# shanjiayao/PTT

Measured on AMD Instinct MI355X. Metric: tracklet frames/sec (hot path: PointNet++ SA stack + Point-Track-Transformer blocks), higher is better.
Workload: dtype f32

## Files before the change

### include/ptt_hip.h

```cpp
#ifndef PTT_HIP_H
#define PTT_HIP_H

#include <stddef.h>
#include <stdint.h>

#ifdef __cplusplus
extern "C" {
#endif

#define PTT_ABI_VERSION 26

enum {
    PTT_OK = 0,
    PTT_EINVAL = -1,
    PTT_EUNSUPPORTED = -2,
    PTT_ELAUNCH = -3,
    PTT_EWORKSPACE = -4
};

typedef void* ptt_stream_t;

int ptt_version(void);
const char* ptt_error_name(int code);
const char* ptt_last_error_string(void);

int ptt_fps_f32(const float* xyz, int B, int N, int npoint, int32_t* idx_out,
                ptt_stream_t stream);
int ptt_fps_ws_f32(const float* xyz, int B, int N, int npoint, int32_t* idx_out, float* workspace,
                   size_t workspace_elems, ptt_stream_t stream);

int ptt_gather_f32(const float* feat, const int32_t* idx, int B, int C, int N, int M,
                   float* out, ptt_stream_t stream);
int ptt_gather_grad_f32(const float* grad_out, const int32_t* idx, int B, int C, int N,
                        int M, float* grad_feat, ptt_stream_t stream);

int ptt_select_centres_f32(const float* xyz, const int32_t* idx, int B, int N, int M, float* new_xyz,
                           int64_t* idx64_out, ptt_stream_t stream);

int ptt_ball_query_f32(const float* new_xyz, const float* xyz, int B, int M, int N,
                       float radius, int nsample, int32_t* idx_out, ptt_stream_t stream);

int ptt_centres_ball_query_f32(const float* xyz, const int32_t* sel, int B, int N, int M, float radius, int nsample,
                               float* new_xyz, int64_t* idx64_out, int32_t* idx_out, ptt_stream_t stream);

int ptt_group_f32(const float* feat, const int32_t* idx, int B, int C, int N, int M,
                  int ns, float* out, ptt_stream_t stream);
int ptt_group_grad_f32(const float* grad_out, const int32_t* idx, int B, int C, int N,
                       int M, int ns, float* grad_feat, ptt_stream_t stream);

size_t ptt_scatter_add_det_workspace(int B, int N, int E);
int ptt_scatter_add_det_f32(const float* src, const int32_t* idx, int B, int C, int N, int E, float* out,
                            void* workspace, size_t workspace_bytes, ptt_stream_t stream);

int ptt_knn_f32(const float* xyz, int B, int N, int k, int32_t* idx_out,
                ptt_stream_t stream);
int ptt_knn_rel_f32(const float* xyz, int B, int N, int k, int32_t* idx_out, float* rel_out,
                    ptt_stream_t stream);

size_t ptt_packed_weight_elems(int Cout, int K);
int ptt_pack_weight_f32(const float* W, int Cout, int K, float* packed,
                        ptt_stream_t stream);
int ptt_pack_weight_rot_f32(const float* W, int Cout, int K, int rot, float* packed,
                            ptt_stream_t stream);

int ptt_linear_f32(const float* X, int rows, int K, int ldx, const float* Wpacked, int Cout,
                   const float* scale, const float* shift, int relu, const float* residual,
                   int ldr, float* out, int ldo, ptt_stream_t stream);

#define PTT_SA_MAX_LAYERS 4

typedef struct ptt_sa_layer {
    const float* Wpacked;
    const float* scale;
    const float* shift;
    int Cin;
    int Cout;
    int relu;
} ptt_sa_layer;

int ptt_rows_mlp_f32(const float* X, int rows, int K, int ldx, const ptt_sa_layer* layers, int n_layers,
                     const float* residual, int ldr, float* out, int ldo, ptt_stream_t stream);

size_t ptt_ball_query_grid_workspace(int B, int N);
int ptt_ball_query_grid_f32(const float* new_xyz, const float* xyz, int B, int M, int N, float radius, int nsample,
                            int32_t* idx_out, void* workspace, size_t workspace_bytes, ptt_stream_t stream);
int ptt_centres_ball_query_grid_f32(const float* xyz, const int32_t* sel, int B, int N, int M, float radius, int nsample,
                                    float* new_xyz, int64_t* idx64_out, int32_t* idx_out, void* workspace, size_t workspace_bytes,
                                    ptt_stream_t stream);
int ptt_fps_ball_knn_f32(const float* xyz, int B, int N, int M, float radius, int nsample, int k, int32_t* inds,
                         int64_t* inds64, float* new_xyz, int32_t* idx, int32_t* knn, float* rel, ptt_stream_t stream);
#define PTT_POINT_JOBS_MAX 4
typedef struct ptt_point_job {
    const float* xyz; const int32_t* centre_sel; const int32_t* point_sel;
    float* new_xyz; int64_t* idx64_out; int32_t* idx_out; float* rel_out;
    int32_t kind, sel_ld, B, Nraw, Npts, M, nsample;
    float radius;
} ptt_point_job;
int ptt_point_jobs_f32(const ptt_point_job* jobs, int n_jobs, ptt_stream_t stream);

#define PTT_ROW_JOBS_MAX 4
typedef struct ptt_row_job {
    const float* X; const float* X2;
    const float* Xmax;
    const float* Wpacked; const float* scale; const float* shift;
    const float* res; const float* res2;
    float* out; float* out2; float* raw;
    const float* rel; const float* w1;
    const float* qkv; const int32_t* knn; const float* pos;
    int32_t rows, K, K1, ldx, ldx2, Cout;
    int32_t act, res_split, ldr, ldr2, out_split, out_col0, ldo, ldo2, ldraw;
    int32_t prologue, epilogue, ldq, q_off, k_off, v_off, ldp, N;
    float sm_scale;
// ... 264 lines not shown
    const float* gamma; const float* beta;
    float* act_a; float* act_b;
    float* running_mean; float* running_var;
    int64_t* num_batches_tracked;
    float momentum;
} ptt_bn_train_tail;
int ptt_bn_stats_train_f32(const float* X, int R, int C, int ldx, float eps, float* mean, float* var, float* invstd,
                           void* workspace, size_t workspace_bytes, const ptt_bn_train_tail* tail, ptt_stream_t stream);
int ptt_bn_finish_partials_train_f32(const double* partial, int chunks, int C, int R, float eps, float* mean, float* var,
                                     float* invstd, const ptt_bn_train_tail* tail, ptt_stream_t stream);
typedef struct ptt_pack_job {
    const float* W;
    int64_t out_offset, stride_out, stride_k;
    int32_t Cout, K;
} ptt_pack_job;
int ptt_pack_weights_f32(const ptt_pack_job* jobs_device, int n_jobs, float* arena, ptt_stream_t stream);
size_t ptt_linear_wgrad2_workspace(int R, int Cout, int Cin);
int ptt_linear_wgrad2_f32(const float* dZ, int ldz, const float* X, int ldx, int R, int Cout, int Cin, float* dW,
                          int accumulate, void* workspace, size_t workspace_bytes, const float* x_scale, const float* x_shift,
                          ptt_stream_t stream);

typedef struct ptt_track_loss_desc {
    const float* seed_cls;
    const float* cls_label;
    const int64_t* search_inds;
    const float* votes;
    const float* reg_label;
    const float* box_data;
    const float* centres;
    const float* pos_weight_seed;
    const float* pos_weight_box;
    int32_t B, N, Ns, M, ld_reg;
    float w_seed_cls, w_seed_reg, w_box_cls, w_box_reg;
} ptt_track_loss_desc;
int ptt_track_losses_f32(const ptt_track_loss_desc* desc, float* out8, float* total , ptt_stream_t stream);
int ptt_track_losses_bwd_f32(const ptt_track_loss_desc* desc, const float* out8, const float* upstream, float* d_seed_cls,
                             float* d_votes, float* d_box_data, ptt_stream_t stream);
typedef struct ptt_adam_tensor {
    float* param;
    float* grad;
    float* exp_avg;
    float* exp_avg_sq;
    int64_t n;
} ptt_adam_tensor;
typedef struct ptt_adam_hyper {
    float beta1, beta2, one_minus_beta1, one_minus_beta2 , eps, step_size, bias2_sqrt,
          weight_decay, max_norm;
    int32_t write_clipped;
} ptt_adam_hyper;
int ptt_adam_chunk_elems(void);
int ptt_adam_clip_step_f32(const ptt_adam_tensor* tensors_device, const int32_t* chunk_tensor_device, const int64_t* chunk_first_device,
                           int n_chunks, const ptt_adam_hyper* hyper, double* partial, size_t partial_elems, float* norm_out,
                           ptt_stream_t stream);
int ptt_adam_clip_step_dev_f32(const ptt_adam_tensor* tensors_device, const int32_t* chunk_tensor_device, const int64_t* chunk_first_device,
                               int n_chunks, const ptt_adam_hyper* hyper_device, int clip, double* partial, size_t partial_elems,
                               float* norm_out, ptt_stream_t stream);
int ptt_unit_rows_f32(const float* x, long long sb, long long sn, long long sc, int B, int n, int C, float eps, float* unit, float* nrm,
                      ptt_stream_t stream);
int ptt_cos_bwd_rows_f32(const float* A, const float* unit, const float* nrm, const float* G, const float* cosm, long long map_sb,
                         long long own, long long other, int m, int B, int n, int C, float* dx, long long sb, long long sn, long long sc,
                         ptt_stream_t stream);
size_t ptt_sa_z0_bnbwd_workspace(long long R, int C);
int ptt_sa_z0_bnbwd_f32(const double* partial, int chunks, const float* G, const float* Z0, const float* rel_rows, const float* mean,
                        const float* invstd, const float* gamma, const float* act_scale, const float* act_shift, long long R, int C,
                        float* dz_out, float* dwx, float* dgamma, float* dbeta, void* workspace, size_t workspace_bytes, ptt_stream_t stream);

typedef struct ptt_grad_job {
    const float* partial;
    int32_t nchunks, reserved;
} ptt_grad_job;
typedef struct ptt_grad_segment {
    int64_t dst;
    int32_t n, cols, ld, job0, njobs, out, vec, reserved;
} ptt_grad_segment;
int ptt_linear_wgrad_partials_f32(const float* dZ, int ldz, const float* X, int ldx, int R, int Cout, int Cin, void* workspace,
                                  size_t workspace_bytes, const float* x_scale, const float* x_shift, int* nchunks, ptt_stream_t stream);
int ptt_linear_wgrad2_partials_f32(const float* dZ, int ldz, const float* X, int ldx, int R, int Cout, int Cin, void* workspace,
                                   size_t workspace_bytes, const float* x_scale, const float* x_shift, int* nchunks, ptt_stream_t stream);
int ptt_colsum_partials_f32(const float* X, int R, int C, int ldx, void* workspace, size_t workspace_bytes, int* nchunks,
                            ptt_stream_t stream);
int ptt_grad_finish_f32(const ptt_grad_segment* segments_device, const ptt_grad_job* jobs_device, const int32_t* blocks_device,
                        int n_blocks, float* flat, ptt_stream_t stream);

int ptt_rows_gemm_rsum16_supported(int rows, int K, int N, int ldx);
int ptt_rows_gemm_rsum16_f32(const float* X, int rows, int K, int ldx, const float* Wpacked, int N, const float* residual, int ldr,
                             float* out, int ldo, float* plain, int ldp, float* gsum, int ldg, ptt_stream_t stream);
int ptt_scatter_rows_csr_sub_f32(const float* g, const int32_t* order, const int32_t* start, int B, int N, int E, int C,
                                 const float* minuend, float* out, ptt_stream_t stream);

int ptt_layernorm_train_fwd_f32(const float* x, int rows, int C, int ldx, const float* weight, const float* bias, float eps,
                                const float* residual, int ldr, float* out, int ldo, float* mean, float* rstd, ptt_stream_t stream);
size_t ptt_layernorm_bwd_workspace(int rows, int C);
int ptt_layernorm_bwd_f32(const float* dy, int ldg, const float* x, int ldx, const float* mean, const float* rstd, const float* weight,
                          int rows, int C, float* dx, int ldd, float* dweight, float* dbias, void* workspace, size_t workspace_bytes,
                          ptt_stream_t stream);
int ptt_rows_gemm_rsum16_heads_supported(int rows, int D, int hd, int ldx);
int ptt_rows_gemm_rsum16_heads_f32(const float* X, int rows, int D, int hd, int ldx, const float* Wpacked, const float* residual, int ldr,
                                   float* out, int ldo, float* plain, int ldp, float* gsum, int ldg, ptt_stream_t stream);

#ifdef __cplusplus
}
#endif
#endif
```

### ptt_amd/_lib.py

```python
import ctypes
import os
import re
from ctypes import Structure, c_char_p, c_double, c_float, c_int, c_int32, c_int64, c_longlong, c_size_t, c_uint32, c_void_p

from .build import HEADER as HEADER_PATH, LIB as LIB_PATH


def _strip_comments(text):
    return re.sub(r"/\*.*?\*/|//[^\n]*", " ", text, flags=re.S)


def parse_defines(text):
    return {n: int(v) for n, v in re.findall(r"^[ \t]*#[ \t]*define[ \t]+(PTT_\w+)[ \t]+(-?\d+)[ \t]*$", _strip_comments(text), re.M)}


CTYPES = {"int": c_int, "int32_t": c_int32, "uint32_t": c_uint32, "int64_t": c_int64, "long long": c_longlong, "size_t": c_size_t,
          "float": c_float, "double": c_double, "ptt_stream_t": c_void_p}


def _ctype(decl, name, is_return=False):
    words = decl.replace("*", " * ").split()
    if not is_return and len(words) > 1 and words[-1] != "*":
        words.pop()
    if "*" in words:
# ... 34 lines not shown

_header = _read_header()
PROTOTYPES = parse_prototypes(_header)
EXPORTS = list(PROTOTYPES)
DEFINES = parse_defines(_header)
ABI_VERSION = DEFINES["PTT_ABI_VERSION"]
PTT_SA_MAX_LAYERS = DEFINES["PTT_SA_MAX_LAYERS"]
PTT_MAX_SEGMENTS = DEFINES["PTT_MAX_SEGMENTS"]
PTT_CROP_JOBS_BY_VALUE_MAX = DEFINES["PTT_CROP_JOBS_BY_VALUE_MAX"]


class CropJob(Structure):
    _fields_ = [("points", c_void_p), ("ld", c_int64),
                ("lo1", c_double * 3), ("hi1", c_double * 3), ("trans", c_double * 3), ("rot", c_double * 9),
                ("lo2", c_double * 3), ("hi2", c_double * 3),
                ("out", c_void_p), ("count", c_void_p), ("n_points", c_int32), ("capacity", c_int32),
                ("label_out", c_void_p), ("ltrans", c_double * 3), ("lrot", c_double * 9), ("llo", c_double * 3), ("lhi", c_double * 3),
                ("append", c_int32), ("reserved", c_int32)]


class RegularizeJob(Structure):
    _fields_ = [("seg", c_void_p * PTT_MAX_SEGMENTS), ("seg_count", c_void_p * PTT_MAX_SEGMENTS),
                ("seg_capacity", c_int32 * PTT_MAX_SEGMENTS), ("out", c_void_p), ("info", c_void_p),
                ("n_seg", c_int32), ("input_size", c_int32)]


class TrackBox(Structure):
    _fields_ = [("center", c_double * 3), ("wlh", c_double * 3), ("quat", c_double * 4)]


class BnTrainTail(Structure):
    _fields_ = [("gamma", c_void_p), ("beta", c_void_p), ("act_a", c_void_p), ("act_b", c_void_p),
                ("running_mean", c_void_p), ("running_var", c_void_p), ("num_batches_tracked", c_void_p), ("momentum", c_float)]


class BnBwdInput(Structure):
    _fields_ = [("g", c_void_p), ("ldg", c_int), ("arg", c_void_p), ("ns", c_int), ("z", c_void_p), ("ldz", c_int),
                ("k1", c_void_p), ("c0", c_void_p), ("c1", c_void_p), ("mean", c_void_p), ("act_a", c_void_p), ("act_b", c_void_p),
                ("dz_out", c_void_p), ("ldd", c_int)]


class PackJob(Structure):
    _fields_ = [("W", c_void_p), ("out_offset", c_int64), ("stride_out", c_int64), ("stride_k", c_int64),
                ("Cout", c_int32), ("K", c_int32)]


class RowJob(Structure):
    _fields_ = [("X", c_void_p), ("X2", c_void_p), ("Xmax", c_void_p), ("Wpacked", c_void_p), ("scale", c_void_p), ("shift", c_void_p),
                ("res", c_void_p), ("res2", c_void_p), ("out", c_void_p), ("out2", c_void_p), ("raw", c_void_p),
                ("rel", c_void_p), ("w1", c_void_p), ("qkv", c_void_p), ("knn", c_void_p), ("pos", c_void_p),
                ("rows", c_int32), ("K", c_int32), ("K1", c_int32), ("ldx", c_int32), ("ldx2", c_int32), ("Cout", c_int32),
                ("act", c_int32), ("res_split", c_int32), ("ldr", c_int32), ("ldr2", c_int32), ("out_split", c_int32),
                ("out_col0", c_int32), ("ldo", c_int32), ("ldo2", c_int32), ("ldraw", c_int32),
                ("prologue", c_int32), ("epilogue", c_int32), ("ldq", c_int32), ("q_off", c_int32), ("k_off", c_int32),
                ("v_off", c_int32), ("ldp", c_int32), ("N", c_int32), ("sm_scale", c_float), ("col_tiles", c_int32),
                ("idx", c_void_p), ("xyz", c_void_p), ("centres", c_void_p), ("wx", c_void_p), ("radius", c_float),
                ("ns", c_int32), ("M", c_int32), ("normalize_xyz", c_int32), ("pro_relu", c_int32)]


class PointJob(Structure):
    _fields_ = [("xyz", c_void_p), ("centre_sel", c_void_p), ("point_sel", c_void_p), ("new_xyz", c_void_p), ("idx64_out", c_void_p),
                ("idx_out", c_void_p), ("rel_out", c_void_p), ("kind", c_int32), ("sel_ld", c_int32), ("B", c_int32),
                ("Nraw", c_int32), ("Npts", c_int32), ("M", c_int32), ("nsample", c_int32), ("radius", c_float)]


class TrackLossDesc(Structure):
    _fields_ = [("seed_cls", c_void_p), ("cls_label", c_void_p), ("search_inds", c_void_p), ("votes", c_void_p), ("reg_label", c_void_p),
                ("box_data", c_void_p), ("centres", c_void_p), ("pos_weight_seed", c_void_p), ("pos_weight_box", c_void_p),
                ("B", c_int32), ("N", c_int32), ("Ns", c_int32), ("M", c_int32), ("ld_reg", c_int32),
                ("w_seed_cls", c_float), ("w_seed_reg", c_float), ("w_box_cls", c_float), ("w_box_reg", c_float)]


class AdamTensor(Structure):
    _fields_ = [("param", c_void_p), ("grad", c_void_p), ("exp_avg", c_void_p), ("exp_avg_sq", c_void_p), ("n", c_int64)]


class GradJob(Structure):
    _fields_ = [("partial", c_void_p), ("nchunks", c_int32), ("reserved", c_int32)]


class GradSegment(Structure):
    _fields_ = [("dst", c_int64), ("n", c_int32), ("cols", c_int32), ("ld", c_int32), ("job0", c_int32), ("njobs", c_int32), ("out", c_int32),
                ("vec", c_int32), ("reserved", c_int32)]


class AdamHyper(Structure):
    _fields_ = [("beta1", c_float), ("beta2", c_float), ("one_minus_beta1", c_float), ("one_minus_beta2", c_float), ("eps", c_float), ("step_size", c_float), ("bias2_sqrt", c_float),
                ("weight_decay", c_float), ("max_norm", c_float), ("write_clipped", c_int32)]


class SaLayer(Structure):
    _fields_ = [("Wpacked", c_void_p), ("scale", c_void_p), ("shift", c_void_p),
                ("Cin", c_int), ("Cout", c_int), ("relu", c_int)]


class SaDesc(Structure):
    _fields_ = [("xyz", c_void_p), ("new_xyz", c_void_p), ("idx", c_void_p), ("feat", c_void_p),
                ("feat_sb", c_int64), ("feat_sc", c_int64), ("feat_sn", c_int64),
                ("out", c_void_p), ("out_sb", c_int64), ("out_sc", c_int64), ("out_sm", c_int64),
                ("B", c_int), ("N", c_int), ("M", c_int), ("nsample", c_int), ("C", c_int),
                ("radius", c_float), ("use_xyz", c_int), ("normalize_xyz", c_int), ("n_layers", c_int),
                ("layers", SaLayer * PTT_SA_MAX_LAYERS),
                ("l0_point_term", c_void_p), ("l0_xyz_weight", c_void_p), ("l0_channels", c_int), ("l0_relu", c_int),
                ("compact_ws", c_void_p), ("compact_ws_bytes", c_size_t)]


class XcorrDesc(Structure):
    _fields_ = [("cos_t", c_void_p), ("P", c_void_p), ("w_sim", c_void_p), ("scale0", c_void_p), ("shift0", c_void_p),
                ("out", c_void_p), ("out_sb", c_int64), ("out_sc", c_int64), ("out_sn", c_int64),
                ("sim_out", c_void_p),
                ("B", c_int), ("Ns", c_int), ("Nt", c_int), ("C0", c_int),
                ("n_layers", c_int), ("layers", SaLayer * PTT_SA_MAX_LAYERS),
                ("split", c_int32), ("out_sh", c_int64), ("search_feat", c_void_p), ("templ_feat", c_void_p),
                ("s_sb", c_int64), ("s_sn", c_int64), ("t_sb", c_int64), ("t_sn", c_int64), ("C", c_int), ("eps", c_float)]


class AttnDesc(Structure):
    _fields_ = [("xyz", c_void_p), ("rel", c_void_p), ("knn", c_void_p), ("qkv", c_void_p),
                ("Wd1p", c_void_p), ("Wd2p", c_void_p), ("bd2", c_void_p),
                ("Wg1p", c_void_p), ("bg1", c_void_p), ("Wg2p", c_void_p), ("bg2", c_void_p),
                ("res", c_void_p), ("attn", c_void_p),
                ("B", c_int), ("N", c_int), ("k", c_int), ("D", c_int), ("order", c_void_p), ("heads", c_int)]


_lib = None


def lib():
    global _lib
    if _lib is None:
        if not os.path.exists(LIB_PATH):
            raise RuntimeError(
                "ptt_amd: %s is missing — build it with `python -m ptt_amd.build` "
                "(hipcc --offload-arch=gfx950); there is no CPU fallback" % LIB_PATH)
        import torch
        try:
            loaded = ctypes.CDLL(LIB_PATH)
        except OSError as e:
            raise RuntimeError("ptt_amd: cannot load %s: %s" % (LIB_PATH, e))
        for name, (restype, argtypes) in PROTOTYPES.items():
            fn = getattr(loaded, name)
            fn.restype, fn.argtypes = restype, argtypes
        if loaded.ptt_version() != ABI_VERSION:
            raise RuntimeError("ptt_amd: %s has ABI version %d, this package expects %d — rebuild it with "
                               "`python -m ptt_amd.build`" % (LIB_PATH, loaded.ptt_version(), ABI_VERSION))
        _lib = loaded
    return _lib


def check(rc, what):
    if rc != 0:
        l = lib()
        raise RuntimeError("%s failed: %s (%s)" % (what, l.ptt_error_name(rc).decode(),
                                                   l.ptt_last_error_string().decode()))
```

### ptt_amd/csrc/point_ops.hip

```cpp
#pragma clang fp contract(off)

#include <limits.h>
#include <stdlib.h>
#include "common.h"

namespace ptt {

__device__ __forceinline__ float sqdist3(float ax, float ay, float az, float bx, float by, float bz) {
    const float dx = ax - bx, dy = ay - by, dz = az - bz;
    return (dx * dx + dy * dy) + dz * dz;
}

__device__ __forceinline__ float knn_dist(float ax, float ay, float az, float bx, float by, float bz) {
    const float d = sqdist3(ax, ay, az, bx, by, bz);
    return d < __builtin_inff() ? d : 3.402823466e+38f;
}

__device__ __forceinline__ float lane_bcast(float v, int src_lane) {
    return __builtin_bit_cast(float, __builtin_amdgcn_readlane(__builtin_bit_cast(int, v), src_lane));
}

typedef float fps_f2 __attribute__((ext_vector_type(2)));


template <int T, int P, bool LX, int ABL = 0>
__global__ __launch_bounds__(T) void fps_kernel(const float* __restrict__ xyz, int N, int npoint,
                                               int32_t* __restrict__ idx_out) {
    constexpr int W = T / 64;
    const int b = blockIdx.x;
    const float* __restrict__ pts = xyz + (size_t)b * N * 3;
    int32_t* __restrict__ out = idx_out + (size_t)b * npoint;
    const int t = threadIdx.x;
    const int lane = t & 63;
    const int wv = t >> 6;

    extern __shared__ int sel_lds[];
    float* xyz_lds = reinterpret_cast<float*>(sel_lds + ((npoint + 3) & ~3));

    float px[P], py[P], pz[P], md[P];
#pragma unroll
    for (int i = 0; i < P; ++i) {
        const int k = t * P + i;
        float x = 0.f, y = 0.f, z = 0.f, m = -1.0f;
        if (k < N) {
            x = pts[3 * k + 0];
            y = pts[3 * k + 1];
            z = pts[3 * k + 2];
            const float mag = (x * x + y * y) + z * z;
            m = (mag > 1e-3f) ? 1e10f : -1.0f;
            if (LX) { xyz_lds[3 * k + 0] = x; xyz_lds[3 * k + 1] = y; xyz_lds[3 * k + 2] = z; }
        }
        px[i] = x; py[i] = y; pz[i] = z; md[i] = m;
    }

    __shared__ __attribute__((aligned(16))) float slots[2][W > 1 ? W : 1][8];

    float lx = pts[0], ly = pts[1], lz = pts[2];
    if (t == 0 && npoint > 0) sel_lds[0] = 0;
    if (LX) __syncthreads();

    for (int j = 1; j < npoint; ++j) {
        float best = -1.0f, bx = 0.f, by = 0.f, bz = 0.f;
        int besti = 0;
        if constexpr ((P % 2) == 0) {
            const fps_f2 lxv = {lx, lx}, lyv = {ly, ly}, lzv = {lz, lz};
#pragma unroll
            for (int i = 0; i < ((ABL & 32) ? 2 : P); i += 2) {
                const fps_f2 dx = fps_f2{px[i], px[i + 1]} - lxv, dy = fps_f2{py[i], py[i + 1]} - lyv,
                             dz = fps_f2{pz[i], pz[i + 1]} - lzv;
                const fps_f2 d = (dx * dx + dy * dy) + dz * dz;
#pragma unroll
                for (int h = 0; h < 2; ++h) {
                    const float m = fminf(md[i + h], d[h]);
                    md[i + h] = m;
                    const bool take = m > best;
                    best = take ? m : best;
                    besti = take ? t * P + i + h : besti;
                    if (!LX) {
                        bx = take ? px[i + h] : bx;
                        by = take ? py[i + h] : by;
                        bz = take ? pz[i + h] : bz;
                    }
                }
            }
        } else {
#pragma unroll
            for (int i = 0; i < P; ++i) {
                const float d = sqdist3(px[i], py[i], pz[i], lx, ly, lz);
                const float m = fminf(md[i], d);
                md[i] = m;
                const bool take = m > best;
                best = take ? m : best;
                besti = take ? t * P + i : besti;
                if (!LX) {
                    bx = take ? px[i] : bx;
                    by = take ? py[i] : by;
                    bz = take ? pz[i] : bz;
                }
            }
        }
        float wmax;
        if constexpr (ABL & 1) wmax = __builtin_amdgcn_readfirstlane(best); else wmax = wave_max_f32_fused(best);
        int src;
        if constexpr (ABL & 2) {
            src = (int)(__builtin_bit_cast(unsigned, wmax) & 63u);
        } else {
            const unsigned long long winners = __ballot(best == wmax);
            src = __ffsll((long long)winners) - 1;
            if constexpr (ABL & 1) src &= 63;
        }
        if constexpr (W == 1) {
            int widx = __builtin_amdgcn_readlane(besti, src);
// ... 2 lines not shown
                lx = (float)widx * 1e-3f; ly = lx; lz = lx;
            } else if constexpr (LX) {
                lx = xyz_lds[3 * widx + 0]; ly = xyz_lds[3 * widx + 1]; lz = xyz_lds[3 * widx + 2];
            } else if (wmax < 0.f) {
                lx = pts[0]; ly = pts[1]; lz = pts[2];
            } else {
                lx = lane_bcast(bx, src); ly = lane_bcast(by, src); lz = lane_bcast(bz, src);
            }
            if (lane == 0) sel_lds[j] = widx;
        } else if constexpr ((ABL & 4) != 0) {
            int gi = __builtin_amdgcn_readlane(besti, src);
            if (wmax < 0.f) gi = 0;
            if constexpr ((ABL & 8) != 0) { lx = (float)gi * 1e-3f; ly = lx; lz = lx; }
            else { lx = xyz_lds[3 * gi + 0]; ly = xyz_lds[3 * gi + 1]; lz = xyz_lds[3 * gi + 2]; }
            if (lane == 0 && wv == 0) sel_lds[j] = gi;
        } else {
            const int par = j & 1;
            if (lane == src) {
                if constexpr (LX) {
                    *reinterpret_cast<float2*>(slots[par][wv]) = make_float2(best, __builtin_bit_cast(float, besti));
                } else {
                    float4* s4 = reinterpret_cast<float4*>(slots[par][wv]);
                    s4[0] = make_float4(best, __builtin_bit_cast(float, besti), bx, by);
                    slots[par][wv][4] = bz;
                }
            }
            if constexpr ((ABL & 16) == 0) __syncthreads();
            float gd, gx = 0.f, gy = 0.f, gz = 0.f;
            int gi;
            if constexpr (W <= 4) {
                gd = -1.0f; gi = 0;
#pragma unroll
                for (int w = 0; w < W; ++w) {
                    if constexpr (LX) {
                        const float2 s2 = *reinterpret_cast<const float2*>(slots[par][w]);
                        const bool take = s2.x > gd;
                        gd = take ? s2.x : gd;
                        gi = take ? __builtin_bit_cast(int, s2.y) : gi;
                    } else {
                        const float4 s4 = *reinterpret_cast<const float4*>(slots[par][w]);
                        const float sz = slots[par][w][4];
                        const bool take = s4.x > gd;
                        gd = take ? s4.x : gd;
                        gi = take ? __builtin_bit_cast(int, s4.y) : gi;
                        gx = take ? s4.z : gx;
                        gy = take ? s4.w : gy;
                        gz = take ? sz : gz;
                    }
                }
            } else {
                if constexpr (LX) {
                    float2 s2 = make_float2(-1.0f, 0.f);
                    if (lane < W) s2 = *reinterpret_cast<const float2*>(slots[par][lane]);
                    gd = wave_max_f32_fused(s2.x);
                    const int sl = __ffsll((long long)__ballot(s2.x == gd)) - 1;
                    gi = __builtin_amdgcn_readlane(__builtin_bit_cast(int, s2.y), sl);
                } else {
                    float4 s4 = make_float4(-1.0f, 0.f, 0.f, 0.f);
                    float sz = 0.f;
                    if (lane < W) { s4 = *reinterpret_cast<const float4*>(slots[par][lane]); sz = slots[par][lane][4]; }
                    gd = wave_max_f32_fused(s4.x);
                    const int sl = __ffsll((long long)__ballot(s4.x == gd)) - 1;
                    gi = __builtin_amdgcn_readlane(__builtin_bit_cast(int, s4.y), sl);
                    gx = lane_bcast(s4.z, sl); gy = lane_bcast(s4.w, sl); gz = lane_bcast(sz, sl);
                }
            }
            if (gd < 0.f) gi = 0;
            if constexpr ((ABL & 16) != 0) gi &= 1023;
            if constexpr ((ABL & 8) != 0) {
                lx = (float)gi * 1e-3f; ly = lx; lz = lx;
            } else if constexpr (LX) {
                lx = xyz_lds[3 * gi + 0]; ly = xyz_lds[3 * gi + 1]; lz = xyz_lds[3 * gi + 2];
            } else {
                if (gd < 0.f) { gx = pts[0]; gy = pts[1]; gz = pts[2]; }
                lx = gx; ly = gy; lz = gz;
            }
            if (t == 0) sel_lds[j] = gi;
        }
    }
    __syncthreads();
    for (int j = t; j < npoint; j += T) out[j] = sel_lds[j];
}

template <int T, int P>
static int launch_fps(const float* xyz, int B, int N, int npoint, int32_t* idx, hipStream_t s) {
    const size_t sel_bytes = (size_t)((npoint + 3) & ~3) * sizeof(int);
    if (sel_bytes + (size_t)N * 12 + 1024 <= 65536 && !dev_switches().fps_plain) {
#ifdef PTT_DEV
        if (const char* e = getenv("PTT_FPS_ABL")) {
            const int abl = atoi(e);
#define PTT_FPS_ABL_CASE(A) if (abl == A) { hipLaunchKernelGGL((fps_kernel<T, P, true, A>), dim3(B), dim3(T), sel_bytes + (size_t)N * 12, s, xyz, N, npoint, idx); return check_launch("fps_kernel(abl)"); }
            PTT_FPS_ABL_CASE(1) PTT_FPS_ABL_CASE(2) PTT_FPS_ABL_CASE(3) PTT_FPS_ABL_CASE(4) PTT_FPS_ABL_CASE(8) PTT_FPS_ABL_CASE(12) PTT_FPS_ABL_CASE(15)
            PTT_FPS_ABL_CASE(16) PTT_FPS_ABL_CASE(32) PTT_FPS_ABL_CASE(47) PTT_FPS_ABL_CASE(7) PTT_FPS_ABL_CASE(24) PTT_FPS_ABL_CASE(40)
#undef PTT_FPS_ABL_CASE
        }
#endif
        hipLaunchKernelGGL((fps_kernel<T, P, true>), dim3(B), dim3(T), sel_bytes + (size_t)N * 12, s, xyz, N, npoint, idx);
        return check_launch("fps_kernel");
    }
    hipLaunchKernelGGL((fps_kernel<T, P, false>), dim3(B), dim3(T), sel_bytes, s, xyz, N, npoint, idx);
    return check_launch("fps_kernel");
}

template <int CPW>
__device__ __forceinline__ void ball_sweep(const float* __restrict__ pts, int N, float r2, int ns, const float (&cx)[CPW],
                                           const float (&cy)[CPW], const float (&cz)[CPW], int ncentres,
                                           int32_t* __restrict__ out0, int lane) {
    int cnt[CPW], first[CPW];
#pragma unroll
    for (int c = 0; c < CPW; ++c) { cnt[c] = (c < ncentres) ? 0 : ns; first[c] = 0; }
    for (int base = 0; base < N; base += 64) {
        const int k = base + lane;
        const bool in = k < N;
        float px = 0.f, py = 0.f, pz = 0.f;
        if (in) { px = pts[3 * k + 0]; py = pts[3 * k + 1]; pz = pts[3 * k + 2]; }
        bool active = false;
#pragma unroll
        for (int c = 0; c < CPW; ++c) {
            if (cnt[c] >= ns) continue;
            const float d = sqdist3(cx[c], cy[c], cz[c], px, py, pz);
            const bool hit = in && d < r2;
            const unsigned long long mask = __ballot(hit);
            if (mask != 0ull) {
                if (cnt[c] == 0) first[c] = base + (__ffsll((long long)mask) - 1);
                const int pos = cnt[c] + __popcll(mask & ((1ull << lane) - 1ull));
                if (hit && pos < ns) out0[(size_t)c * ns + pos] = k;
                cnt[c] += __popcll(mask);
            }
            active = active || cnt[c] < ns;
        }
        if (!active) break;
    }
#pragma unroll
    for (int c = 0; c < CPW; ++c) {
        if (c >= ncentres) break;
        const int fill = (cnt[c] > 0) ? first[c] : 0;
        for (int s = cnt[c] + lane; s < ns; s += 64) out0[(size_t)c * ns + s] = fill;
    }
}

template <int CPW>
__global__ __launch_bounds__(256) void ball_query_kernel(const float* __restrict__ new_xyz,
                                                         const float* __restrict__ xyz, int BM, int M, int N,
                                                         float r2, int ns, int32_t* __restrict__ idx_out) {
    const int centre = (blockIdx.x * 4 + (threadIdx.x >> 6)) * CPW;
    if (centre >= BM) return;
    const int lane = threadIdx.x & 63;
    const int b = centre / M;
    float cx[CPW], cy[CPW], cz[CPW];
    const int nc = min(CPW, BM - centre);
#pragma unroll
    for (int c = 0; c < CPW; ++c) {
        const int cc = centre + (c < nc ? c : 0);
        cx[c] = new_xyz[(size_t)cc * 3 + 0]; cy[c] = new_xyz[(size_t)cc * 3 + 1]; cz[c] = new_xyz[(size_t)cc * 3 + 2];
    }
    ball_sweep<CPW>(xyz + (size_t)b * N * 3, N, r2, ns, cx, cy, cz, nc, idx_out + (size_t)centre * ns, lane);
}

template <int CPW>
__global__ __launch_bounds__(256) void centres_ball_query_kernel(const float* __restrict__ xyz, const int32_t* __restrict__ sel,
                                                                 int BM, int M, int N, float r2, int ns,
                                                                 float* __restrict__ new_xyz, long long* __restrict__ idx64,
                                                                 int32_t* __restrict__ idx_out) {
    const int centre = (blockIdx.x * 4 + (threadIdx.x >> 6)) * CPW;
    if (centre >= BM) return;
    const int lane = threadIdx.x & 63;
// ... 691 lines not shown
            const int s0 = cstart[c0], s1 = cstart[c0 + (x1 - x0) + 1];
            for (int e = s0 + lane; e < s1; e += 64) {
                const int k = cpts[e];
                const float d = sqdist3(cx, cy, cz, pts[3 * k], pts[3 * k + 1], pts[3 * k + 2]);
                if (d < r2) atomicOr(&bits[k >> 5], 1u << (k & 31));
            }
        }
    }
    __builtin_amdgcn_wave_barrier();
    asm volatile("s_waitcnt lgkmcnt(0)" ::: "memory");
    int32_t* __restrict__ out = idx_out + (size_t)centre * ns;
    int cnt = 0, first = 0;
    for (int w0 = 0; w0 < words && cnt < ns; w0 += 64) {
        const int w = w0 + lane;
        unsigned v = w < words ? bits[w] : 0u;
        const int mine = __popc(v);
        int incl = mine;
#pragma unroll
        for (int off = 1; off < 64; off <<= 1) { const int u = __shfl_up(incl, off, 64); if (lane >= off) incl += u; }
        const int total = __shfl(incl, 63, 64);
        if (total == 0) continue;
        if (cnt == 0) {
            const unsigned long long any = __ballot(mine > 0);
            const int fl = __ffsll((long long)any) - 1;
            const unsigned fv = __shfl(v, fl, 64);
            first = ((w0 + fl) << 5) + (__ffs(fv) - 1);
        }
        int pos = cnt + incl - mine;
        while (v != 0u && pos < ns) {
            const int bit = __ffs(v) - 1;
            out[pos++] = (w << 5) + bit;
            v &= v - 1u;
        }
        cnt += total;
    }
    const int have = cnt < ns ? cnt : ns;
    const int fill = cnt > 0 ? first : 0;
    for (int s2 = have + lane; s2 < ns; s2 += 64) out[s2] = fill;
}

}

using namespace ptt;

extern "C" int ptt_fps_f32(const float* xyz, int B, int N, int npoint, int32_t* idx_out, ptt_stream_t stream) {
    if (B < 0 || N <= 0 || npoint < 0) return fail(PTT_EINVAL, "ptt_fps_f32: B=%d N=%d npoint=%d", B, N, npoint);
    if (B == 0 || npoint == 0) return PTT_OK;
    if (!xyz || !idx_out) return fail(PTT_EINVAL, "ptt_fps_f32: null pointer");
    if (npoint > 15360) return fail(PTT_EUNSUPPORTED, "ptt_fps_f32: npoint=%d exceeds the LDS index buffer (15360)", npoint);
    hipStream_t s = as_stream(stream);
    if (N <= 64) return launch_fps<64, 1>(xyz, B, N, npoint, idx_out, s);
    if (N <= 128) return launch_fps<64, 2>(xyz, B, N, npoint, idx_out, s);
    if (N <= 256) return launch_fps<64, 4>(xyz, B, N, npoint, idx_out, s);
    if (N <= 512) {
        if (const int T = dev_switches().fps_t) {
            if (T == 256) return launch_fps<256, 2>(xyz, B, N, npoint, idx_out, s);
            if (T == 128) return launch_fps<128, 4>(xyz, B, N, npoint, idx_out, s);
            if (T == 512) return launch_fps<512, 1>(xyz, B, N, npoint, idx_out, s);
        }
        return launch_fps<64, 8>(xyz, B, N, npoint, idx_out, s);
    }
    if (N <= 1024) {
        if (const int T = dev_switches().fps_t) {
            if (T == 64) return launch_fps<64, 16>(xyz, B, N, npoint, idx_out, s);
            if (T == 128) return launch_fps<128, 8>(xyz, B, N, npoint, idx_out, s);
            if (T == 512) return launch_fps<512, 2>(xyz, B, N, npoint, idx_out, s);
        }
        return launch_fps<256, 4>(xyz, B, N, npoint, idx_out, s);
    }
    if (N <= 2048) {
        if (const int T = dev_switches().fps_t) {
            if (T == 512) return launch_fps<512, 4>(xyz, B, N, npoint, idx_out, s);
            if (T == 1024) return launch_fps<1024, 2>(xyz, B, N, npoint, idx_out, s);
            if (T == 128) return launch_fps<128, 16>(xyz, B, N, npoint, idx_out, s);
        }
        return launch_fps<256, 8>(xyz, B, N, npoint, idx_out, s);
    }
    if (N <= 4096) return launch_fps<512, 8>(xyz, B, N, npoint, idx_out, s);
    if (N <= 8192) return launch_fps<1024, 8>(xyz, B, N, npoint, idx_out, s);
    if (N <= 16384) return launch_fps<1024, 16>(xyz, B, N, npoint, idx_out, s);
    return fail(PTT_EUNSUPPORTED, "ptt_fps_f32: N=%d exceeds the register-resident limit 16384 (use ptt_fps_ws_f32)", N);
}

extern "C" int ptt_spatial_order_f32(const float* xyz, int B, int N, int32_t* order, ptt_stream_t stream) {
    if (B < 0 || N <= 0) return fail(PTT_EINVAL, "ptt_spatial_order_f32: B=%d N=%d", B, N);
    if (B == 0) return PTT_OK;
    if (!xyz || !order) return fail(PTT_EINVAL, "ptt_spatial_order_f32: null pointer");
    if (N > 8192 || (long long)B * N > INT_MAX) return fail(PTT_EUNSUPPORTED, "ptt_spatial_order_f32: N=%d (at most 8192 points per cloud are sorted in LDS)", N);
    int P = 2;
    while (P < N) P <<= 1;
    const int lds = P * (int)sizeof(unsigned long long);
    if (int rc = set_lds_limit(reinterpret_cast<const void*>(spatial_order_kernel), lds)) return rc;
    hipLaunchKernelGGL(spatial_order_kernel, dim3(B), dim3(1024), lds, as_stream(stream), xyz, N, P, order);
    return check_launch("spatial_order_kernel");
}

extern "C" int ptt_fps_ws_f32(const float* xyz, int B, int N, int npoint, int32_t* idx_out, float* workspace, size_t workspace_elems,
                              ptt_stream_t stream) {
    if (B < 0 || N <= 0 || npoint < 0) return fail(PTT_EINVAL, "ptt_fps_ws_f32: B=%d N=%d npoint=%d", B, N, npoint);
    if (B == 0 || npoint == 0) return PTT_OK;
    if (!xyz || !idx_out) return fail(PTT_EINVAL, "ptt_fps_ws_f32: null pointer");
    if ((long long)N * 3 > INT_MAX) return fail(PTT_EUNSUPPORTED, "ptt_fps_ws_f32: N=%d", N);
    if (!workspace || workspace_elems < (size_t)B * N)
        return fail(PTT_EWORKSPACE, "ptt_fps_ws_f32: %zu floats of workspace needed", (size_t)B * N);
    hipLaunchKernelGGL(fps_ws_kernel, dim3(B), dim3(1024), 0, as_stream(stream), xyz, N, npoint, workspace, idx_out);
    return check_launch("fps_ws_kernel");
}

static int ball_cpw(int BM, int M) {
    const int force = dev_switches().ball_cpw;
    if (force == 1 || (M & 3) != 0) return 1;
    if (force == 8 && (M & 7) == 0) return 8;
    if (force == 4) return 4;
    return BM >= 4 * 256 * 8 ? 4 : 1;
}

extern "C" int ptt_ball_query_f32(const float* new_xyz, const float* xyz, int B, int M, int N, float radius,
                                  int nsample, int32_t* idx_out, ptt_stream_t stream) {
    if (B < 0 || M < 0 || N <= 0 || nsample <= 0)
        return fail(PTT_EINVAL, "ptt_ball_query_f32: B=%d M=%d N=%d nsample=%d", B, M, N, nsample);
    if (B == 0 || M == 0) return PTT_OK;
    if (!new_xyz || !xyz || !idx_out) return fail(PTT_EINVAL, "ptt_ball_query_f32: null pointer");
    const float r2 = radius * radius;
    const int BM = B * M;
    const int cpw = ball_cpw(BM, M);
    if (cpw == 8)
        hipLaunchKernelGGL((ball_query_kernel<8>), dim3((BM / 8 + 3) / 4), dim3(256), 0, as_stream(stream), new_xyz, xyz, BM, M,
                           N, r2, nsample, idx_out);
    else if (cpw == 4)
        hipLaunchKernelGGL((ball_query_kernel<4>), dim3((BM / 4 + 3) / 4), dim3(256), 0, as_stream(stream), new_xyz, xyz, BM, M,
                           N, r2, nsample, idx_out);
    else
        hipLaunchKernelGGL((ball_query_kernel<1>), dim3((BM + 3) / 4), dim3(256), 0, as_stream(stream), new_xyz, xyz, BM, M,
                           N, r2, nsample, idx_out);
    return check_launch("ball_query_kernel");
}

extern "C" int ptt_gather_f32(const float* feat, const int32_t* idx, int B, int C, int N, int M, float* out,
                              ptt_stream_t stream) {
    if (B < 0 || C < 0 || N <= 0 || M < 0) return fail(PTT_EINVAL, "ptt_gather_f32: bad sizes");
    const size_t total = (size_t)B * C * M;
    if (total == 0) return PTT_OK;
    if (!feat || !idx || !out) return fail(PTT_EINVAL, "ptt_gather_f32: null pointer");
    hipLaunchKernelGGL(gather_kernel, dim3(grid_for(total, 256)), dim3(256), 0, as_stream(stream), feat, idx, C, N, M,
                       out, total);
    return check_launch("gather_kernel");
}

extern "C" int ptt_select_centres_f32(const float* xyz, const int32_t* idx, int B, int N, int M, float* new_xyz,
                                      int64_t* idx64_out, ptt_stream_t stream) {
    if (B < 0 || N <= 0 || M < 0 || (!idx && M > N)) return fail(PTT_EINVAL, "ptt_select_centres_f32: B=%d N=%d M=%d", B, N, M);
    const size_t total = (size_t)B * M;
    if (total == 0) return PTT_OK;
    if (!xyz || !new_xyz) return fail(PTT_EINVAL, "ptt_select_centres_f32: null pointer");
    hipLaunchKernelGGL(select_centres_kernel, dim3(grid_for(total, 256)), dim3(256), 0, as_stream(stream), xyz, idx, N, M,
                       new_xyz, reinterpret_cast<long long*>(idx64_out), total);
    return check_launch("select_centres_kernel");
}

extern "C" int ptt_gather_grad_f32(const float* grad_out, const int32_t* idx, int B, int C, int N, int M,
                                   float* grad_feat, ptt_stream_t stream) {
    if (B < 0 || C < 0 || N <= 0 || M < 0) return fail(PTT_EINVAL, "ptt_gather_grad_f32: bad sizes");
    const size_t nout = (size_t)B * C * N;
    if (nout == 0) return PTT_OK;
    if (!grad_feat) return fail(PTT_EINVAL, "ptt_gather_grad_f32: null pointer");
    if (hipMemsetAsync(grad_feat, 0, nout * sizeof(float), as_stream(stream)) != hipSuccess)
// ... 216 lines not shown
```

### ptt_amd/csrc/train_ops.hip

```cpp
#include <math.h>
#include "common.h"

namespace ptt {

typedef float f32x4t __attribute__((ext_vector_type(4)));
typedef float f32x16t __attribute__((ext_vector_type(16)));

constexpr int ST_ROWS = 2048;

template <int MODE>
__global__ __launch_bounds__(256) void col_stats_kernel(const float* __restrict__ X, const float* __restrict__ Act,
                                                        const float* __restrict__ Z, const float* __restrict__ mean,
                                                        const float* __restrict__ invstd, int R, int C, int ldx, int lda,
                                                        int ldz, double* __restrict__ partial) {
    __shared__ double red[2][4][64];
    const int lane = threadIdx.x & 63, rg = threadIdx.x >> 6;
    const int r0 = blockIdx.x * ST_ROWS, r1 = min(R, r0 + ST_ROWS);
    for (int cg = 0; cg * 64 < C; ++cg) {
        const int c = cg * 64 + lane;
        double s0 = 0.0, s1 = 0.0;
        if (c < C) {
            float mu = 0.f, is = 0.f;
            if (MODE == 1) { mu = mean[c]; is = invstd[c]; }
            for (int r = r0 + rg; r < r1; r += 4) {
// ... 575 lines not shown
        const float sa = act_a ? act_a[c] : 1.f, sb = act_a ? act_b[c] : 0.f;
        float m = act_a ? fmaxf(__builtin_fmaf(p[0], sa, sb), 0.f) : p[0];
        int a = 0;
        for (int k = 1; k < ns; ++k) {
            float v = p[(size_t)k * ldx];
            if (act_a) v = fmaxf(__builtin_fmaf(v, sa, sb), 0.f);
            if (v > m) { m = v; a = k; }
        }
        out[(size_t)g * ldo + c] = m;
        arg[(size_t)g * C + c] = a;
    }
}

__global__ __launch_bounds__(256) void pool_select_kernel(const float* __restrict__ pmax, const float* __restrict__ pmin,
                                                          const int32_t* __restrict__ amax, const int32_t* __restrict__ amin,
                                                          const float* __restrict__ act_a, const float* __restrict__ act_b, size_t total,
                                                          int C, float* __restrict__ out, int32_t* __restrict__ arg) {
    for (size_t e = (size_t)blockIdx.x * 256 + threadIdx.x; e < total; e += (size_t)gridDim.x * 256) {
        const int c = (int)(e % C);
        const float a = act_a[c], b = act_b[c];
        const float y = a > 0.f ? pmax[e] : pmin[e];
        out[e] = fmaxf(__builtin_fmaf(y, a, b), 0.f);
        arg[e] = a > 0.f ? amax[e] : (a < 0.f ? amin[e] : 0);
    }
}

__global__ __launch_bounds__(256) void pool_rows_bwd_kernel(const float* __restrict__ dOut, int ldo, const int32_t* __restrict__ arg,
                                                            int G, int ns, int C, float* __restrict__ dX, int ldx) {
    const size_t total = (size_t)G * ns * C;
    for (size_t e = (size_t)blockIdx.x * 256 + threadIdx.x; e < total; e += (size_t)gridDim.x * 256) {
        const size_t row = e / C;
        const int c = (int)(e - row * C);
        const int g = (int)(row / ns), k = (int)(row - (size_t)g * ns);
        dX[row * ldx + c] = (arg[(size_t)g * C + c] == k) ? dOut[(size_t)g * ldo + c] : 0.f;
    }
}

constexpr int WG_KC = 32;
constexpr int WG_LD = 132;
constexpr int WG_ROWS = 4096;
constexpr int WG_MIN_ROWS = 64;

template <bool VEC>
__device__ __forceinline__ void wg_fetch(const float* __restrict__ P, int ld, int r0, int rmax, int c0, int cmax, int t,
                                         f32x4t (&st)[4]) {
#pragma unroll
    for (int i = 0; i < 4; ++i) {
        const int e = t + i * 256;
        const int r = r0 + (e >> 5), c = c0 + ((e & 31) << 2);
        f32x4t v = {0.f, 0.f, 0.f, 0.f};
        if (r < rmax) {
            const float* src = P + (size_t)r * ld + c;
            if (VEC && c + 3 < cmax) {
                v = *reinterpret_cast<const f32x4t*>(src);
            } else {
#pragma unroll
                for (int q = 0; q < 4; ++q)
                    if (c + q < cmax) v[q] = src[q];
            }
        }
        st[i] = v;
    }
}
__device__ __forceinline__ void wg_stage(float* S, int t, const f32x4t (&st)[4]) {
#pragma unroll
    for (int i = 0; i < 4; ++i) {
        const int e = t + i * 256;
        *reinterpret_cast<f32x4t*>(S + (e >> 5) * WG_LD + ((e & 31) << 2)) = st[i];
    }
}

__device__ __forceinline__ void wg_act(f32x4t (&st)[4], const float* __restrict__ xa, const float* __restrict__ xb, int c0, int cmax,
                                       int t) {
    const int c = c0 + ((t & 31) << 2);
    if (c + 3 < cmax) {
        const f32x4t a4 = *reinterpret_cast<const f32x4t*>(xa + c), b4 = *reinterpret_cast<const f32x4t*>(xb + c);
#pragma unroll
        for (int i = 0; i < 4; ++i)
#pragma unroll
            for (int q = 0; q < 4; ++q) st[i][q] = fmaxf(__builtin_fmaf(st[i][q], a4[q], b4[q]), 0.f);
    }
}

template <bool VZ, bool VX, int NS = 1>
__global__ __launch_bounds__(256, 2) void linear_wgrad_kernel(const float* __restrict__ dZ, int ldz, const float* __restrict__ X,
                                                              int ldx, int R, int Cout, int Cin, int nbi, int chunk_rows,
                                                              float* __restrict__ partial, const float* __restrict__ xa,
                                                              const float* __restrict__ xb, int narrow_o = 0, int narrow_i = 0) {
    extern __shared__ __attribute__((aligned(16))) float wg_smem[];
    constexpr int WG_BUF = WG_KC * WG_LD;
#define As(b) (wg_smem + (b) * WG_BUF)
#define Bs(b) (wg_smem + (2 + (b)) * WG_BUF)
    const int t = threadIdx.x, lane = t & 63, w = t >> 6, half = lane >> 5, col = lane & 31;
    const int bo = blockIdx.x / nbi, bi = blockIdx.x - bo * nbi;
    const int o0 = bo * 128, i0 = bi * 128;
    const int r_begin = blockIdx.y * chunk_rows, r_end = min(R, r_begin + chunk_rows);
    int wo = (w >> 1) * 64, wi = (w & 1) * 64;
    int sidx = 0;
    if constexpr (NS > 1) {
        if (narrow_o) { sidx = w >> 1; wo = 0; }
        if (narrow_i) { sidx = sidx * 2 + (w & 1); wi = 0; }
        sidx = __builtin_amdgcn_readfirstlane(sidx);
    }
    f32x16t acc[2][2];
#pragma unroll
    for (int a = 0; a < 2; ++a)
#pragma unroll
        for (int b = 0; b < 2; ++b)
#pragma unroll
            for (int r = 0; r < 16; ++r) acc[a][b][r] = 0.f;
    f32x4t sa[4], sb[4];
    wg_fetch<VZ>(dZ, ldz, r_begin, r_end, o0, Cout, t, sa);
    wg_fetch<VX>(X, ldx, r_begin, r_end, i0, Cin, t, sb);
    if (xa) wg_act(sb, xa, xb, i0, Cin, t);
    wg_stage(As(0), t, sa);
    wg_stage(Bs(0), t, sb);
    __syncthreads();
    int buf = 0;
    for (int r0 = r_begin; r0 < r_end; r0 += WG_KC) {
        const bool more = r0 + WG_KC < r_end;
        if (more) {
            wg_fetch<VZ>(dZ, ldz, r0 + WG_KC, r_end, o0, Cout, t, sa);
            wg_fetch<VX>(X, ldx, r0 + WG_KC, r_end, i0, Cin, t, sb);
            if (xa) wg_act(sb, xa, xb, i0, Cin, t);
        }
        const float* A = As(buf) + (half + sidx * (WG_KC / NS)) * WG_LD + wo + col;
        const float* B = Bs(buf) + (half + sidx * (WG_KC / NS)) * WG_LD + wi + col;
        float fa[2][2], fb[2][2];
        fa[0][0] = A[0]; fa[0][1] = A[32]; fb[0][0] = B[0]; fb[0][1] = B[32];
#pragma unroll
        for (int j = 0; j < WG_KC / 2 / NS; ++j) {
            const int s = j & 1;
            if (j + 1 < WG_KC / 2 / NS) {
                fa[s ^ 1][0] = A[2 * (j + 1) * WG_LD]; fa[s ^ 1][1] = A[2 * (j + 1) * WG_LD + 32];
                fb[s ^ 1][0] = B[2 * (j + 1) * WG_LD]; fb[s ^ 1][1] = B[2 * (j + 1) * WG_LD + 32];
            }
            __builtin_amdgcn_sched_barrier(0);
            acc[0][0] = __builtin_amdgcn_mfma_f32_32x32x2f32(fa[s][0], fb[s][0], acc[0][0], 0, 0, 0);
            acc[0][1] = __builtin_amdgcn_mfma_f32_32x32x2f32(fa[s][0], fb[s][1], acc[0][1], 0, 0, 0);
            acc[1][0] = __builtin_amdgcn_mfma_f32_32x32x2f32(fa[s][1], fb[s][0], acc[1][0], 0, 0, 0);
            acc[1][1] = __builtin_amdgcn_mfma_f32_32x32x2f32(fa[s][1], fb[s][1], acc[1][1], 0, 0, 0);
            __builtin_amdgcn_sched_barrier(0);
        }
        if (more) {
            wg_stage(As(buf ^ 1), t, sa);
            wg_stage(Bs(buf ^ 1), t, sb);
        }
        __syncthreads();
        buf ^= 1;
    }
#undef As
#undef Bs
    if constexpr (NS > 1) {
        float* slot = wg_smem + w * 4096;
#pragma unroll
        for (int a = 0; a < 2; ++a)
#pragma unroll
            for (int b = 0; b < 2; ++b)
#pragma unroll
                for (int r = 0; r < 16; ++r) slot[((a * 2 + b) * 16 + r) * 64 + lane] = acc[a][b][r];
        __syncthreads();
        if (sidx != 0) return;
        const int step = (NS == 4) ? 1 : (narrow_i ? 1 : 2);
        float* P = partial + (size_t)blockIdx.y * Cout * Cin;
        for (int a = 0; a < 2; ++a)
            for (int b = 0; b < 2; ++b) {
                const int ci = i0 + wi + b * 32 + col;
#pragma unroll
                for (int r = 0; r < 16; ++r) {
                    const int e = ((a * 2 + b) * 16 + r) * 64 + lane;
                    float v = slot[e];
                    for (int k = 1; k < NS; ++k) v += wg_smem[(w + k * step) * 4096 + e];
                    const int co = o0 + wo + a * 32 + (r & 3) + 8 * (r >> 2) + 4 * half;
                    if (co < Cout && ci < Cin) P[(size_t)co * Cin + ci] = v;
                }
            }
        return;
    }
    float* P = partial + (size_t)blockIdx.y * Cout * Cin;
#pragma unroll
    for (int a = 0; a < 2; ++a)
#pragma unroll
        for (int b = 0; b < 2; ++b) {
            const int ci = i0 + wi + b * 32 + col;
#pragma unroll
            for (int r = 0; r < 16; ++r) {
                const int co = o0 + wo + a * 32 + (r & 3) + 8 * (r >> 2) + 4 * half;
                if (co < Cout && ci < Cin) P[(size_t)co * Cin + ci] = acc[a][b][r];
            }
        }
}

__global__ __launch_bounds__(256) void colsum_partial_scalar_kernel(const float* __restrict__ X, int ldx, int R, int C, int rows_per_chunk,
                                                                    float* __restrict__ partial) {
    __shared__ float red[4][64];
    const int c = blockIdx.y * 64 + (threadIdx.x & 63), rg = threadIdx.x >> 6;
    const int r0 = blockIdx.x * rows_per_chunk, r1 = min(R, r0 + rows_per_chunk);
    float acc = 0.f;
    if (c < C)
        for (int r = r0 + rg; r < r1; r += 4) acc += X[(size_t)r * ldx + c];
    red[rg][threadIdx.x & 63] = acc;
    __syncthreads();
    if (rg == 0 && c < C) partial[(size_t)blockIdx.x * C + c] = ((red[0][threadIdx.x] + red[1][threadIdx.x]) + red[2][threadIdx.x]) + red[3][threadIdx.x];
}

constexpr int WK_ROWS = 256;
template <int K>
__global__ __launch_bounds__(256) void wgrad_smallk_kernel(const float* __restrict__ dZ, int ldz, const float* __restrict__ X, int ldx,
                                                           int R, int C, float* __restrict__ partial) {
    __shared__ float red[256][4 * K];
    const int Cq = C >> 2, span = Cq < 256 ? Cq : 256, RG = 256 / span;
    const int q0 = threadIdx.x % span, rg = threadIdx.x / span;
    const int r0 = blockIdx.x * WK_ROWS, r1 = min(R, r0 + WK_ROWS);
    for (int qb = 0; qb < Cq; qb += span) {
        const int q = qb + q0;
        float acc[4][K];
#pragma unroll
        for (int j = 0; j < 4; ++j)
#pragma unroll
            for (int k = 0; k < K; ++k) acc[j][k] = 0.f;
        if (q < Cq && rg < RG) {
            for (int r = r0 + rg; r < r1; r += RG) {
                const f32x4t g = *reinterpret_cast<const f32x4t*>(dZ + (size_t)r * ldz + 4 * q);
                float xv[K];
#pragma unroll
                for (int k = 0; k < K; ++k) xv[k] = X[(size_t)r * ldx + k];
#pragma unroll
                for (int j = 0; j < 4; ++j)
#pragma unroll
                    for (int k = 0; k < K; ++k) acc[j][k] = __builtin_fmaf(g[j], xv[k], acc[j][k]);
            }
        }
#pragma unroll
        for (int j = 0; j < 4; ++j)
#pragma unroll
            for (int k = 0; k < K; ++k) red[threadIdx.x][j * K + k] = acc[j][k];
        __syncthreads();
        if (rg == 0 && q < Cq) {
#pragma unroll
            for (int j = 0; j < 4; ++j)
#pragma unroll
                for (int k = 0; k < K; ++k) {
                    float t = 0.f;
                    for (int g2 = 0; g2 < RG; ++g2) t += red[g2 * span + q0][j * K + k];
                    partial[((size_t)blockIdx.x * C + 4 * q + j) * K + k] = t;
                }
        }
        __syncthreads();
    }
}

constexpr int CS_ROWS = 128;
__global__ __launch_bounds__(256) void colsum_partial_kernel(const float* __restrict__ X, int ldx, int R, int C, int rows_per_chunk,
                                                             float* __restrict__ partial) {
    __shared__ f32x4t red[4][64];
    const int q = blockIdx.y * 64 + (threadIdx.x & 63), rg = threadIdx.x >> 6;
    const int r0 = blockIdx.x * rows_per_chunk, r1 = min(R, r0 + rows_per_chunk);
    f32x4t acc = {0.f, 0.f, 0.f, 0.f};
    if (4 * q < C) {
        int r = r0 + rg;
        for (; r + 12 < r1; r += 16) {
            const f32x4t a = *reinterpret_cast<const f32x4t*>(X + (size_t)r * ldx + 4 * q);
            const f32x4t b = *reinterpret_cast<const f32x4t*>(X + (size_t)(r + 4) * ldx + 4 * q);
            const f32x4t c = *reinterpret_cast<const f32x4t*>(X + (size_t)(r + 8) * ldx + 4 * q);
            const f32x4t d = *reinterpret_cast<const f32x4t*>(X + (size_t)(r + 12) * ldx + 4 * q);
#pragma unroll
            for (int k = 0; k < 4; ++k) acc[k] = (((acc[k] + a[k]) + b[k]) + c[k]) + d[k];
        }
        for (; r < r1; r += 4) {
            const f32x4t a = *reinterpret_cast<const f32x4t*>(X + (size_t)r * ldx + 4 * q);
#pragma unroll
            for (int k = 0; k < 4; ++k) acc[k] += a[k];
        }
    }
    red[rg][threadIdx.x & 63] = acc;
    __syncthreads();
    if (rg == 0 && 4 * q < C) {
        f32x4t t = red[0][threadIdx.x];
#pragma unroll
        for (int g = 1; g < 4; ++g)
#pragma unroll
            for (int k = 0; k < 4; ++k) t[k] += red[g][threadIdx.x][k];
        *reinterpret_cast<f32x4t*>(partial + (size_t)blockIdx.x * C + 4 * q) = t;
    }
}

template <int OUT>
__global__ __launch_bounds__(256) void wgrad_finish_kernel(const float* __restrict__ partial, int nchunks, size_t n, int accumulate,
                                                           float* __restrict__ dW) {
    constexpr int G = 256 / OUT;
    __shared__ float part[G][OUT];
    const int lane = threadIdx.x % OUT, g = threadIdx.x / OUT;
    for (size_t base = (size_t)blockIdx.x * OUT; base < n; base += (size_t)gridDim.x * OUT) {
        const size_t e = base + lane;
        float s = 0.f;
        if (e < n)
            for (int k = g; k < nchunks; k += G) s += partial[(size_t)k * n + e];
        part[g][lane] = s;
        __syncthreads();
        if (g == 0 && e < n) {
            float tot = part[0][lane];
            for (int q = 1; q < G; ++q) tot += part[q][lane];
            dW[e] = accumulate ? dW[e] + tot : tot;
        }
        __syncthreads();
    }
}

__global__ __launch_bounds__(256) void grad_finish_kernel(const ptt_grad_segment* __restrict__ segs, const ptt_grad_job* __restrict__ jobs,
                                                          const int32_t* __restrict__ blocks, float* __restrict__ flat) {
    __shared__ f32x4t part[256];
    const ptt_grad_segment sg = segs[blocks[2 * blockIdx.x]];
    const int OUT = sg.out, G = 256 / OUT;
    const int lane = threadIdx.x % OUT, g = threadIdx.x / OUT;
    const int e = (blocks[2 * blockIdx.x + 1] + lane) * (sg.vec ? 4 : 1);
    f32x4t s = {0.f, 0.f, 0.f, 0.f};
    if (e < sg.n) {
        int kbase = 0;
        for (int j = 0; j < sg.njobs; ++j) {
            const ptt_grad_job jb = jobs[sg.job0 + j];
            int c = g - kbase % G;
            if (c < 0) c += G;
            if (sg.vec) {
                const float* pe = jb.partial + e;
                const size_t step = (size_t)G * sg.n;
                for (; c + 3 * G < jb.nchunks; c += 4 * G) {
                    const float* p0 = pe + (size_t)c * sg.n;
                    const f32x4t v0 = *reinterpret_cast<const f32x4t*>(p0), v1 = *reinterpret_cast<const f32x4t*>(p0 + step),
                                 v2 = *reinterpret_cast<const f32x4t*>(p0 + 2 * step), v3 = *reinterpret_cast<const f32x4t*>(p0 + 3 * step);
#pragma unroll
                    for (int x = 0; x < 4; ++x) s[x] = (((s[x] + v0[x]) + v1[x]) + v2[x]) + v3[x];
                }
                for (; c < jb.nchunks; c += G) {
                    const f32x4t v = *reinterpret_cast<const f32x4t*>(pe + (size_t)c * sg.n);
#pragma unroll
                    for (int x = 0; x < 4; ++x) s[x] += v[x];
                }
            } else {
                for (; c < jb.nchunks; c += G) s[0] += jb.partial[(size_t)c * sg.n + e];
            }
            kbase += jb.nchunks;
        }
    }
    part[g * OUT + lane] = s;
    __syncthreads();
    if (g == 0 && e < sg.n) {
        f32x4t tot = part[lane];
        for (int q = 1; q < G; ++q)
#pragma unroll
            for (int x = 0; x < 4; ++x) tot[x] += part[q * OUT + lane][x];
        const int row = e / sg.cols, col = e - row * sg.cols;
        float* d = flat + sg.dst + (long long)row * sg.ld + col;
        if (sg.vec) {
            f32x4t o = *reinterpret_cast<const f32x4t*>(d);
#pragma unroll
            for (int x = 0; x < 4; ++x) o[x] += tot[x];
            *reinterpret_cast<f32x4t*>(d) = o;
        } else {
            *d += tot[0];
        }
    }
}

__global__ __launch_bounds__(256) void gather_rows_kernel(const float* __restrict__ src, const int32_t* __restrict__ idx, int N,
                                                          int E, int C, float* __restrict__ out) {
    const int Cq = C >> 2, span = Cq < 256 ? Cq : 256, RG = 256 / span;
    const int q0 = threadIdx.x % span, rg = threadIdx.x / span;
// ... 750 lines not shown
extern "C" int ptt_scatter_rows_csr_sub_f32(const float* g, const int32_t* order, const int32_t* start, int B, int N, int E, int C,
                                            const float* minuend, float* out, ptt_stream_t stream) {
    return scatter_rows_run(g, order, start, B, N, E, C, out, minuend, 1, stream);
}

static int pt_train_check(const char* what, int B, int N, int k, int D, const void* p0, const void* p1, const void* p2, const void* p3) {
    if (B < 0 || N <= 0 || D <= 0 || (D & 3)) return fail(PTT_EINVAL, "%s: B=%d N=%d D=%d (D %% 4)", what, B, N, D);
    if (k != 16) return fail(PTT_EUNSUPPORTED, "%s: k=%d (16 neighbours is instantiated)", what, k);
    if (B > 0 && (!p0 || !p1 || !p2 || !p3)) return fail(PTT_EINVAL, "%s: null pointer", what);
    return PTT_OK;
}

extern "C" int ptt_pt_pair_input_f32(const float* q, const float* kf, const int32_t* knn, const float* pos, int B, int N, int k,
                                     int D, float* t, ptt_stream_t stream) {
    if (int rc = pt_train_check("ptt_pt_pair_input_f32", B, N, k, D, q, kf, knn, pos)) return rc;
    if (B == 0) return PTT_OK;
    if (!t) return fail(PTT_EINVAL, "ptt_pt_pair_input_f32: null pointer");
    const long long pts = (long long)B * N;
    hipLaunchKernelGGL((pair_input_kernel<16>), dim3(ew_grid((size_t)pts * (D >> 2))), dim3(256), 0, as_stream(stream), q, kf, knn, pos, N,
                       D, pts, t, D, D);
    return check_launch("pair_input_kernel");
}

extern "C" int ptt_pt_pair_input_ld_f32(const float* q, int ldq, const float* kf, int ldk, const int32_t* knn, const float* pos, int B,
                                        int N, int k, int D, float* t, ptt_stream_t stream) {
    if (int rc = pt_train_check("ptt_pt_pair_input_ld_f32", B, N, k, D, q, kf, knn, pos)) return rc;
    if (ldq < D || ldk < D || (ldq & 3) || (ldk & 3)) return fail(PTT_EINVAL, "ptt_pt_pair_input_ld_f32: ldq=%d ldk=%d", ldq, ldk);
    if (B == 0) return PTT_OK;
    if (!t) return fail(PTT_EINVAL, "ptt_pt_pair_input_ld_f32: null pointer");
    const long long pts = (long long)B * N;
    hipLaunchKernelGGL((pair_input_kernel<16>), dim3(ew_grid((size_t)pts * (D >> 2))), dim3(256), 0, as_stream(stream), q, kf, knn, pos, N,
                       D, pts, t, ldq, ldk);
    return check_launch("pair_input_kernel");
}

extern "C" int ptt_pt_attn_fwd_ld_f32(const float* a, const float* vf, int ldv, const int32_t* knn, const float* pos, int B, int N, int k,
                                      int D, float scale, float* attn, float* res, ptt_stream_t stream) {
    if (int rc = pt_train_check("ptt_pt_attn_fwd_ld_f32", B, N, k, D, a, vf, knn, pos)) return rc;
    if (ldv < D || (ldv & 3)) return fail(PTT_EINVAL, "ptt_pt_attn_fwd_ld_f32: ldv=%d", ldv);
    if (B == 0) return PTT_OK;
    if (!res) return fail(PTT_EINVAL, "ptt_pt_attn_fwd_ld_f32: null pointer");
    const long long pts = (long long)B * N;
    hipLaunchKernelGGL((attn_fwd_kernel<16>), dim3(ew_grid((size_t)pts * (D >> 2))), dim3(256), 0, as_stream(stream), a, vf, knn, pos, N, D,
                       pts, scale, attn, res, ldv);
    return check_launch("attn_fwd_kernel");
}

extern "C" int ptt_pt_attn_train_fwd_f32(const float* a, const float* vf, const int32_t* knn, const float* pos, int B, int N, int k,
                                         int D, float scale, float* attn, float* res, ptt_stream_t stream) {
    if (int rc = pt_train_check("ptt_pt_attn_train_fwd_f32", B, N, k, D, a, vf, knn, pos)) return rc;
    if (B == 0) return PTT_OK;
    if (!attn || !res) return fail(PTT_EINVAL, "ptt_pt_attn_train_fwd_f32: null pointer");
    const long long pts = (long long)B * N;
    hipLaunchKernelGGL((attn_fwd_kernel<16>), dim3(ew_grid((size_t)pts * (D >> 2))), dim3(256), 0, as_stream(stream), a, vf, knn, pos, N, D,
                       pts, scale, attn, res, D);
    return check_launch("attn_fwd_kernel");
}

extern "C" int ptt_pt_attn_train_bwd_f32(const float* attn, const float* vf, const int32_t* knn, const float* pos, const float* dres,
                                         int B, int N, int k, int D, float scale, float* da, float* dvp, ptt_stream_t stream) {
    if (int rc = pt_train_check("ptt_pt_attn_train_bwd_f32", B, N, k, D, attn, vf, knn, pos)) return rc;
    if (B == 0) return PTT_OK;
    if (!dres || !da || !dvp) return fail(PTT_EINVAL, "ptt_pt_attn_train_bwd_f32: null pointer");
    const long long pts = (long long)B * N;
    hipLaunchKernelGGL((attn_bwd_kernel<16>), dim3(ew_grid((size_t)pts * (D >> 2))), dim3(256), 0, as_stream(stream), attn, vf, knn, pos,
                       dres, N, D, pts, scale, da, dvp);
    return check_launch("attn_bwd_kernel");
}

static inline bool wgrad_smallk_ok(int Cout, int Cin) { return Cin >= 1 && Cin <= 4 && (Cout & 3) == 0; }

static inline int colsum_rows_per_chunk(int R, int C) {
    const int colblocks = (C + 255) / 256;
    int chunks = 512 / colblocks;
    int rows = (R + chunks - 1) / chunks;
    if (rows < CS_ROWS) rows = CS_ROWS;
    return (rows + 3) / 4 * 4;
}
extern "C" size_t ptt_colsum_workspace(int R, int C) {
    if (R <= 0 || C <= 0) return 0;
    const int rows = colsum_rows_per_chunk(R, C);
    return (size_t)((R + rows - 1) / rows) * (size_t)C * sizeof(float);
}
static int colsum_run(const float* X, int R, int C, int ldx, float* out, void* ws, size_t ws_bytes, int* nchunks_out, ptt_stream_t stream) {
    if (R <= 0 || C <= 0 || ldx < C) return fail(PTT_EINVAL, "ptt_colsum_f32: R=%d C=%d ldx=%d", R, C, ldx);
    if (!X || (!out && !nchunks_out)) return fail(PTT_EINVAL, "ptt_colsum_f32: null pointer");
    const int rows = colsum_rows_per_chunk(R, C), nch = (R + rows - 1) / rows;
    hipStream_t s2 = as_stream(stream);
    if ((nch > 1 || !out) && (!ws || ws_bytes < ptt_colsum_workspace(R, C))) return fail(PTT_EWORKSPACE, "ptt_colsum_f32: workspace too small");
    float* part = (nch == 1 && out) ? out : static_cast<float*>(ws);
    const bool vec = !(C & 3) && !(ldx & 3) && !((reinterpret_cast<uintptr_t>(X) | reinterpret_cast<uintptr_t>(part)) & 15);
    if (vec) hipLaunchKernelGGL(colsum_partial_kernel, dim3(nch, (C / 4 + 63) / 64), dim3(256), 0, s2, X, ldx, R, C, rows, part);
    else hipLaunchKernelGGL(colsum_partial_scalar_kernel, dim3(nch, (C + 63) / 64), dim3(256), 0, s2, X, ldx, R, C, rows, part);
    if (nch > 1 && out) launch_wgrad_finish(part, nch, (size_t)C, 0, out, s2);
    if (nchunks_out) *nchunks_out = nch;
    return check_launch("colsum_partial_kernel");
}
extern "C" int ptt_colsum_f32(const float* X, int R, int C, int ldx, float* out, void* ws, size_t ws_bytes, ptt_stream_t stream) {
    if (!out) return fail(PTT_EINVAL, "ptt_colsum_f32: null pointer");
    return colsum_run(X, R, C, ldx, out, ws, ws_bytes, nullptr, stream);
}
extern "C" int ptt_colsum_partials_f32(const float* X, int R, int C, int ldx, void* ws, size_t ws_bytes, int* nchunks, ptt_stream_t stream) {
    if (!nchunks) return fail(PTT_EINVAL, "ptt_colsum_partials_f32: null pointer");
    return colsum_run(X, R, C, ldx, nullptr, ws, ws_bytes, nchunks, stream);
}

extern "C" size_t ptt_linear_wgrad_workspace(int R, int Cout, int Cin) {
    if (R <= 0 || Cout <= 0 || Cin <= 0) return 0;
    if (wgrad_smallk_ok(Cout, Cin)) return (size_t)((R + WK_ROWS - 1) / WK_ROWS) * (size_t)Cout * Cin * sizeof(float);
    const int rows = wgrad_stream_ok(R, Cout, Cin, Cout, Cin) ? wgrad_stream_rows(R) : wgrad_chunk_rows(R, Cout, Cin);
    return (size_t)((R + rows - 1) / rows) * (size_t)Cout * Cin * sizeof(float);
}

static int linear_wgrad_run(const float* dZ, int ldz, const float* X, int ldx, int R, int Cout, int Cin, float* dW,
                            int accumulate, void* ws, size_t ws_bytes, const float* x_scale, const float* x_shift,
                            int* nchunks_out, ptt_stream_t stream) {
    if (x_scale && (!x_shift || (Cin & 3) || ((reinterpret_cast<uintptr_t>(x_scale) | reinterpret_cast<uintptr_t>(x_shift)) & 15)))
        return fail(PTT_EINVAL, "ptt_linear_wgrad_f32: the input transform needs Cin %% 4 == 0 and 16-byte aligned scale / shift");
    if (R <= 0 || Cout <= 0 || Cin <= 0 || ldz < Cout || ldx < Cin)
        return fail(PTT_EINVAL, "ptt_linear_wgrad_f32: R=%d Cout=%d Cin=%d ldz=%d ldx=%d", R, Cout, Cin, ldz, ldx);
    if (!dZ || !X || (!dW && !nchunks_out)) return fail(PTT_EINVAL, "ptt_linear_wgrad_f32: null pointer");
    if (!ws || ws_bytes < ptt_linear_wgrad_workspace(R, Cout, Cin))
        return fail(PTT_EWORKSPACE, "ptt_linear_wgrad_f32: workspace too small");
    if (wgrad_smallk_ok(Cout, Cin) && !x_scale && (ldz & 3) == 0 && (reinterpret_cast<uintptr_t>(dZ) & 15) == 0) {
        const int nch = (R + WK_ROWS - 1) / WK_ROWS;
        hipStream_t s2 = as_stream(stream);
        float* part = static_cast<float*>(ws);
        if (Cin == 1) hipLaunchKernelGGL((wgrad_smallk_kernel<1>), dim3(nch), dim3(256), 0, s2, dZ, ldz, X, ldx, R, Cout, part);
        else if (Cin == 2) hipLaunchKernelGGL((wgrad_smallk_kernel<2>), dim3(nch), dim3(256), 0, s2, dZ, ldz, X, ldx, R, Cout, part);
        else if (Cin == 3) hipLaunchKernelGGL((wgrad_smallk_kernel<3>), dim3(nch), dim3(256), 0, s2, dZ, ldz, X, ldx, R, Cout, part);
        else hipLaunchKernelGGL((wgrad_smallk_kernel<4>), dim3(nch), dim3(256), 0, s2, dZ, ldz, X, ldx, R, Cout, part);
        if (dW) launch_wgrad_finish(part, nch, (size_t)Cout * Cin, accumulate, dW, s2);
        if (nchunks_out) *nchunks_out = nch;
        return check_launch("wgrad_smallk_kernel");
    }
    if (wgrad_stream_ok(R, Cout, Cin, ldz, ldx)) {
        const int rows = wgrad_stream_rows(R), nch = (R + rows - 1) / rows;
        hipStream_t s2 = as_stream(stream);
        if (int rc = launch_wgrad_stream(dZ, ldz, X, ldx, R, Cout, Cin, rows, static_cast<float*>(ws), x_scale, x_shift, s2)) return rc;
        if (dW) launch_wgrad_finish(static_cast<const float*>(ws), nch, (size_t)Cout * Cin, accumulate, dW, s2);
        if (nchunks_out) *nchunks_out = nch;
        return check_launch("wgrad_stream_kernel");
    }
    const int rows = wgrad_chunk_rows(R, Cout, Cin);
    const int nchunks = (R + rows - 1) / rows;
    const int nbo = (Cout + 127) / 128, nbi = (Cin + 127) / 128;
    hipStream_t s = as_stream(stream);
    const int lds = 4 * WG_KC * WG_LD * (int)sizeof(float);
    const bool vz = (ldz & 3) == 0 && (reinterpret_cast<uintptr_t>(dZ) & 15) == 0;
    const bool vx = (ldx & 3) == 0 && (reinterpret_cast<uintptr_t>(X) & 15) == 0;
    const int narrow_o = (Cout <= 64), narrow_i = (Cin <= 64);
    const int ns = (narrow_o ? 2 : 1) * (narrow_i ? 2 : 1);
#define PTT_WGRAD_CASE(VZ, VX)                                                                                        \
    if (vz == VZ && vx == VX) {                                                                                       \
        if (ns == 1) {                                                                                                \
            if (int rc = set_lds_limit(reinterpret_cast<const void*>(linear_wgrad_kernel<VZ, VX, 1>), lds)) return rc; \
            hipLaunchKernelGGL((linear_wgrad_kernel<VZ, VX, 1>), dim3(nbo * nbi, nchunks), dim3(256), lds, s, dZ, ldz, X, ldx, R, Cout, \
                               Cin, nbi, rows, static_cast<float*>(ws), x_scale, x_shift, 0, 0);                      \
        } else if (ns == 2) {                                                                                         \
            if (int rc = set_lds_limit(reinterpret_cast<const void*>(linear_wgrad_kernel<VZ, VX, 2>), lds)) return rc; \
            hipLaunchKernelGGL((linear_wgrad_kernel<VZ, VX, 2>), dim3(nbo * nbi, nchunks), dim3(256), lds, s, dZ, ldz, X, ldx, R, Cout, \
                               Cin, nbi, rows, static_cast<float*>(ws), x_scale, x_shift, narrow_o, narrow_i);        \
        } else {                                                                                                      \
            if (int rc = set_lds_limit(reinterpret_cast<const void*>(linear_wgrad_kernel<VZ, VX, 4>), lds)) return rc; \
            hipLaunchKernelGGL((linear_wgrad_kernel<VZ, VX, 4>), dim3(nbo * nbi, nchunks), dim3(256), lds, s, dZ, ldz, X, ldx, R, Cout, \
                               Cin, nbi, rows, static_cast<float*>(ws), x_scale, x_shift, narrow_o, narrow_i);        \
        }                                                                                                             \
    }
    PTT_WGRAD_CASE(true, true) PTT_WGRAD_CASE(true, false) PTT_WGRAD_CASE(false, true) PTT_WGRAD_CASE(false, false)
#undef PTT_WGRAD_CASE
    if (dW) launch_wgrad_finish(static_cast<const float*>(ws), nchunks, (size_t)Cout * Cin, accumulate, dW, s);
    if (nchunks_out) *nchunks_out = nchunks;
    return check_launch("linear_wgrad_kernel");
}
extern "C" int ptt_linear_wgrad_f32(const float* dZ, int ldz, const float* X, int ldx, int R, int Cout, int Cin, float* dW,
                                    int accumulate, void* ws, size_t ws_bytes, const float* x_scale, const float* x_shift,
                                    ptt_stream_t stream) {
    if (!dW) return fail(PTT_EINVAL, "ptt_linear_wgrad_f32: null pointer");
    return linear_wgrad_run(dZ, ldz, X, ldx, R, Cout, Cin, dW, accumulate, ws, ws_bytes, x_scale, x_shift, nullptr, stream);
}
extern "C" int ptt_linear_wgrad_partials_f32(const float* dZ, int ldz, const float* X, int ldx, int R, int Cout, int Cin, void* ws,
                                             size_t ws_bytes, const float* x_scale, const float* x_shift, int* nchunks,
                                             ptt_stream_t stream) {
    if (!nchunks) return fail(PTT_EINVAL, "ptt_linear_wgrad_partials_f32: null pointer");
    return linear_wgrad_run(dZ, ldz, X, ldx, R, Cout, Cin, nullptr, 0, ws, ws_bytes, x_scale, x_shift, nchunks, stream);
}

extern "C" int ptt_grad_finish_f32(const ptt_grad_segment* segments_device, const ptt_grad_job* jobs_device, const int32_t* blocks_device,
                                   int n_blocks, float* flat, ptt_stream_t stream) {
    if (n_blocks < 0) return fail(PTT_EINVAL, "ptt_grad_finish_f32: n_blocks=%d", n_blocks);
    if (n_blocks == 0) return PTT_OK;
    if (!segments_device || !jobs_device || !blocks_device || !flat || (reinterpret_cast<uintptr_t>(flat) & 15))
        return fail(PTT_EINVAL, "ptt_grad_finish_f32: null table or a gradient buffer that is not 16-byte aligned");
    hipLaunchKernelGGL(grad_finish_kernel, dim3(n_blocks), dim3(256), 0, as_stream(stream), segments_device, jobs_device, blocks_device, flat);
    return check_launch("grad_finish_kernel");
}

extern "C" int ptt_bn_finish_partials_train_f32(const double* partial, int chunks, int C, int R, float eps, float* mean, float* var,
                                                float* invstd, const ptt_bn_train_tail* tail, ptt_stream_t stream) {
    if (chunks <= 0 || C <= 0 || R <= 0 || !partial || !mean || !var || !invstd)
        return fail(PTT_EINVAL, "ptt_bn_finish_partials_f32: chunks=%d C=%d R=%d", chunks, C, R);
    BnTail bt;
    if (int rc = bn_tail_from(tail, C, &bt, "ptt_bn_finish_partials_train_f32")) return rc;
    hipLaunchKernelGGL((col_stats_finish2_kernel<0>), dim3(C), dim3(256), 0, as_stream(stream), partial, chunks, C, R, eps, mean, var,
                       invstd, bt);
    return check_launch("col_stats_finish2_kernel");
}

extern "C" int ptt_bn_finish_partials_f32(const double* partial, int chunks, int C, int R, float eps, float* mean, float* var,
                                          float* invstd, ptt_stream_t stream) {
    return ptt_bn_finish_partials_train_f32(partial, chunks, C, R, eps, mean, var, invstd, nullptr, stream);
}

extern "C" int ptt_bn_sums_partials_f64(const double* partial, int chunks, int C, int R, double* sums, ptt_stream_t stream) {
    if (chunks <= 0 || C <= 0 || R <= 0 || !partial || !sums) return fail(PTT_EINVAL, "ptt_bn_sums_partials_f64: chunks=%d C=%d R=%d", chunks, C, R);
    hipLaunchKernelGGL(col_sums_finish_kernel, dim3(C), dim3(256), 0, as_stream(stream), partial, chunks, C, sums, (double)R);
    return check_launch("col_sums_finish_kernel");
}

extern "C" int ptt_bn_update_running_f32(const float* mean, const float* var, const double* count, float momentum, int C,
                                         float* running_mean, float* running_var, int64_t* num_batches_tracked, ptt_stream_t stream) {
    if (C <= 0 || !mean || !var || !count || !running_mean || !running_var) return fail(PTT_EINVAL, "ptt_bn_update_running_f32: C=%d or null pointer", C);
    hipLaunchKernelGGL(bn_running_update_kernel, dim3((C + 255) / 256), dim3(256), 0, as_stream(stream), mean, var, count, momentum, C,
                       running_mean, running_var, reinterpret_cast<long long*>(num_batches_tracked));
    return check_launch("bn_running_update_kernel");
}

static inline int xcorr_z0_grid(long long rows, int C, bool stats) {
    const int Cq = C >> 2, RG = 256 / (Cq < 256 ? Cq : 256);
    long long grid = (rows + RG * 8 - 1) / (RG * 8);
    const long long cap = stats ? 4096 : 16384;
    return (int)(grid > cap ? cap : grid);
}
static int xcorr_z0_launch(const float* P, const float* cos_t, const float* w_sim, int B, int n2, int n1, int C, float* z0, double* stats,
                           ptt_stream_t stream) {
    if (B <= 0 || n2 <= 0 || n1 <= 0 || C <= 0 || (C & 3)) return fail(PTT_EINVAL, "ptt_xcorr_z0_f32: B=%d n2=%d n1=%d C=%d", B, n2, n1, C);
    if (!P || !cos_t || !w_sim || !z0 || !vec4_ok(P, C, C) || !vec4_ok(z0, C, C) || !vec4_ok(w_sim, 4, 4))
        return fail(PTT_EINVAL, "ptt_xcorr_z0_f32: null or misaligned pointer");
    const long long rows = (long long)B * n2 * n1;
    hipLaunchKernelGGL(xcorr_z0_kernel, dim3((unsigned)xcorr_z0_grid(rows, C, stats != nullptr)), dim3(256), 0, as_stream(stream), P, cos_t,
                       w_sim, n2, n1, C, rows, z0, stats);
    return check_launch("xcorr_z0_kernel");
}
extern "C" int ptt_xcorr_z0_f32(const float* P, const float* cos_t, const float* w_sim, int B, int n2, int n1, int C, float* z0,
                                ptt_stream_t stream) {
    return xcorr_z0_launch(P, cos_t, w_sim, B, n2, n1, C, z0, nullptr, stream);
}
extern "C" int ptt_xcorr_z0_stat_chunks(int B, int n2, int n1, int C) {
    if (B <= 0 || n2 <= 0 || n1 <= 0 || C <= 0 || (C & 3) || C > 1024) return 0;
    return xcorr_z0_grid((long long)B * n2 * n1, C, true);
}
extern "C" int ptt_xcorr_z0_stats_f32(const float* P, const float* cos_t, const float* w_sim, int B, int n2, int n1, int C, float* z0,
                                      double* stats_partial, size_t partial_elems, ptt_stream_t stream) {
    const int chunks = ptt_xcorr_z0_stat_chunks(B, n2, n1, C);
    if (!chunks) return fail(PTT_EUNSUPPORTED, "ptt_xcorr_z0_stats_f32: B=%d n2=%d n1=%d C=%d (C %% 4 == 0, at most 1024 channels)", B, n2, n1, C);
    if (!stats_partial || partial_elems < (size_t)chunks * 2 * (size_t)C)
// ... 154 lines not shown
```

### ptt_amd/models/backbones_3d/pointnet2_backbone.py

```python
from typing import List

import torch
import torch.nn as nn

from ... import graph_policy, ops, train_ops
from .pointnet2 import pointnet2_modules


class PointNet2BackboneLight(nn.Module):
    def __init__(self, model_cfg, input_channels, **kwargs):
        super().__init__()
        self.model_cfg = model_cfg
        input_channels -= 3
        self.num_points_each_layer = []
        self.SA_modules = nn.ModuleList()
        sa = self.model_cfg.SA_CONFIG
        for k in range(len(sa.RADIUS)):
            mlps = list(sa.MLPS[k])
            if k == 0:
                mlps[0] = input_channels
            self.SA_modules.append(pointnet2_modules.PointnetSAModuleVotes(
                radius=sa.RADIUS[k], nsample=sa.NSAMPLE[k], mlp=mlps,
                use_xyz=sa.get('USE_XYZ', True), normalize_xyz=sa.get('NORMALIZE_XYZ', True),
                sample_method=sa.SAMPLE_METHOD[k]))
        self.cov_final = nn.Conv1d(256, 256, kernel_size=1)
        self.num_point_features = sa.MLPS[-1][-1]
        self._cov_cache = None
        self.seed_knn = 16
        self.overlap_branches = True
        self._side_stream = None

    @staticmethod
    def _break_up_pc(pc):
        xyz = pc[..., 0:3].contiguous()
        features = pc[..., 3:].contiguous() if pc.size(-1) > 3 else None
        return xyz, features

    def _cov_final(self, features):
        if not features.is_cuda:
            return self.cov_final(features)
        if self.training:
            if features.dtype != torch.float32:
                return self.cov_final(features)
            return train_ops.rows_linear(self.cov_final, features.transpose(1, 2)).transpose(1, 2)
        if ops.autograd_recording(self.cov_final, features) or features.dtype != torch.float32:
            ops.note_unfused('PointNet2BackboneLight.cov_final', 'autograd is recording or input is not float32')
            return self.cov_final(features)
        w, b = self.cov_final.weight, self.cov_final.bias
        key = (w.data_ptr(), w._version, b.data_ptr(), b._version)
        if self._cov_cache is None or self._cov_cache[0] != key:
            self._cov_cache = (key, ops.pack_weight(w), b.detach().float().contiguous())
            ops.publish_params(w.device)
        rows = features.transpose(1, 2)
        out = ops.linear(rows, self._cov_cache[1], w.shape[0], None, self._cov_cache[2])
        return out.transpose(1, 2)

    def _arange64(self, xyz, n):
        key = (xyz.size(0), n, str(xyz.device))
        cache = self.__dict__.setdefault('_arange_cache', {})
        if key not in cache:
            cache[key] = torch.arange(n, dtype=torch.int64, device=xyz.device).repeat(xyz.size(0), 1)
            ops.publish_params(xyz.device, replaced=False)
        return cache[key]

    def branch_forward(self, pts, npoints: List, inds0=None, want_knn=0, compact_levels=()):
        xyz, features = self._break_up_pc(pts)
        sa = self.model_cfg.SA_CONFIG
        one_frame = (not self.training and xyz.is_cuda and features is None and len(self.SA_modules) == 3
                     and xyz.shape[0] * npoints[0] <= 4 * ops.ONE_FRAME_MAX_POINTS
                     and self.SA_modules[0].sample_method == 'fps'
                     and all(m.sample_method in ('rs', 'sequence') for m in self.SA_modules[1:])
                     and npoints[0] >= npoints[1] >= npoints[2] and (not want_knn or npoints[2] <= 128)
                     and all(m._fusable(xyz, None) for m in self.SA_modules[:1]))
        knn = None
        if one_frame:
            from .pointnet2 import pointnet2_utils
            xyz = xyz.contiguous()
            if inds0 is None:
                inds0 = pointnet2_utils.furthest_point_sample(xyz, npoints[0])
            inds0 = inds0.to(torch.int32).contiguous()
            levels, inds64, knn = ops.sa_levels_point_jobs(xyz, inds0, list(npoints), list(sa.RADIUS), list(sa.NSAMPLE),
                                                           knn_k=want_knn)
            seq = [None, self._arange64(xyz, npoints[1]), self._arange64(xyz, npoints[2])]
            xyz, features, inds0 = self.SA_modules[0](xyz=xyz, features=features, npoint=npoints[0], inds=inds0,
                                                      pre=(levels[0][0], levels[0][1], inds64))
            xyz, features, inds1 = self.SA_modules[1](xyz=xyz, features=features, npoint=npoints[1],
                                                      pre=(levels[1][0], levels[1][1], seq[1]))
            xyz, features, inds2 = self.SA_modules[2](xyz=xyz, features=features, npoint=npoints[2],
                                                      pre=(levels[2][0], levels[2][1], seq[2]))
        else:
            xyz, features, inds0 = self.SA_modules[0](xyz=xyz, features=features, npoint=npoints[0], inds=inds0)
            xyz, features, inds1 = self.SA_modules[1](xyz=xyz, features=features, npoint=npoints[1], compact=1 in compact_levels)
            xyz, features, inds2 = self.SA_modules[2](xyz=xyz, features=features, npoint=npoints[2], compact=2 in compact_levels)
        point_features = self._cov_final(features)
        assert inds1.dtype == inds2.dtype == torch.int64, 'index type must be int64, not {}'.format(inds2.dtype)
        if all(m.sample_method in ('rs', 'sequence') for m in self.SA_modules[1:]) and inds0.shape[1] >= npoints[2]:
            inds = inds0[:, :npoints[2]]
        else:
            inds = inds0.gather(1, inds1).gather(1, inds2)
        if want_knn:
            return xyz, point_features, inds, knn
        return xyz, point_features, inds

    def sample(self, search_points, template_points):
        from .pointnet2 import pointnet2_utils
        sa = self.model_cfg.SA_CONFIG
        assert sa.SAMPLE_METHOD[0] == 'fps'
        return (pointnet2_utils.furthest_point_sample(search_points[..., 0:3].contiguous(), sa.NPOINTS_SEARCH[0]),
                pointnet2_utils.furthest_point_sample(template_points[..., 0:3].contiguous(), sa.NPOINTS_TEMPLATE[0]))

    def forward_branches(self, search_points, template_points, inds=None):
        sa = self.model_cfg.SA_CONFIG
        i_s, i_t = inds if inds is not None else (None, None)
        last = (len(self.SA_modules) - 1,) if (search_points.is_cuda and not self.training) else ()
        if not (self.overlap_branches and search_points.is_cuda and not self.training):
            r = self.branch_forward(search_points, sa.NPOINTS_SEARCH, i_s, want_knn=self.seed_knn, compact_levels=last)
            t_seeds, t_feats, t_inds = self.branch_forward(template_points, sa.NPOINTS_TEMPLATE, i_t)
        else:
            if self._side_stream is None or self._side_stream.device != search_points.device:
                self._side_stream = torch.cuda.Stream(device=search_points.device)
            main = torch.cuda.current_stream(search_points.device)
            side = graph_policy.branch(main, self._side_stream)
            with torch.cuda.stream(side):
                t_seeds, t_feats, t_inds = self.branch_forward(template_points, sa.NPOINTS_TEMPLATE, i_t)
            r = self.branch_forward(search_points, sa.NPOINTS_SEARCH, i_s, want_knn=self.seed_knn, compact_levels=last)
            graph_policy.join(main, side)
            if side is not main:
                for t in (t_seeds, t_feats, t_inds, template_points):
                    t.record_stream(main)
        s_seeds, s_feats, s_inds = r[:3]
        s_knn = r[3] if len(r) > 3 else None
        out = {'search_seeds': s_seeds, 'search_feats': s_feats, 'search_inds': s_inds,
               'template_seeds': t_seeds, 'template_feats': t_feats, 'template_inds': t_inds}
        if s_knn is not None:
            out['search_seeds_knn'] = s_knn
        return out

    def forward(self, batch_dict):
        batch_dict.update(self.forward_branches(batch_dict['search_points'], batch_dict['template_points'],
                                                batch_dict.pop('fps_inds', None)))
        batch_dict.pop('search_points')
        batch_dict.pop('template_points')
        return batch_dict
```

### ptt_amd/ops.py

```python
import contextlib
import ctypes
import os

import torch

from . import _lib
from ._lib import AttnDesc, SaDesc, SaLayer, XcorrDesc


def _stream():
    return ctypes.c_void_p(torch.cuda.current_stream().cuda_stream)


_timing = None


def start_kernel_timing(names):
    global _timing
    _timing = {n: [] for n in names}


def stop_kernel_timing():
    global _timing
    t, _timing = _timing, None
# ... 40 lines not shown
    return False


param_generation = 0


def publish_params(device, replaced=True):
    global param_generation
    if replaced:
        param_generation += 1
    if device.type == 'cuda' and not torch.cuda.is_current_stream_capturing():
        torch.cuda.current_stream(device).synchronize()


def drop_params():
    global param_generation
    param_generation += 1


class StateWatch(object):

    def __init__(self, module):
        self.tensors = list(module.parameters()) + list(module.buffers())
        self.mark()

    def _key(self):
        return list(map(torch.Tensor.data_ptr, self.tensors)), [t._version for t in self.tensors]

    def mark(self):
        self.generation, self.key = param_generation, self._key()

    def changed(self):
        return param_generation != self.generation or self._key() != self.key


def require_finite(*tensors):
    bad = [k for k, t in enumerate(tensors) if t is not None and t.is_floating_point() and not bool(torch.isfinite(t).all())]
    if bad:
        raise ValueError("non-finite values in tensor(s) %s" % ", ".join("#%d %s" % (k, tuple(tensors[k].shape)) for k in bad))


def _chk(t, name, dtype, ndim=None):
    if not isinstance(t, torch.Tensor):
        raise TypeError("%s must be a torch.Tensor" % name)
    if not t.is_cuda:
        raise RuntimeError("%s must be a device (HIP) tensor — CPU tensors are not supported" % name)
    if t.dtype != dtype:
        raise RuntimeError("%s must be %s, got %s" % (name, dtype, t.dtype))
    if not t.is_contiguous():
        raise RuntimeError("%s must be contiguous" % name)
    if ndim is not None and t.dim() != ndim:
        raise RuntimeError("%s must have %d dimensions, got %s" % (name, ndim, tuple(t.shape)))
    return t


def _ptr(t):
    return ctypes.c_void_p(t.data_ptr()) if t is not None else ctypes.c_void_p(0)


_UNTIMED = contextlib.nullcontext()


def _launch(name, device, *args, timed=None):
    with torch.cuda.device(device), (_timed(timed) if timed else _UNTIMED):
        rc = getattr(_lib.lib(), name)(*args, _stream())
    if rc:
        _lib.check(rc, name)


def _host(name, *args):
    return getattr(_lib.lib(), name)(*args)


def _host_checked(name, *args):
    _lib.check(_host(name, *args), name)


def _workspace(query, device, *dims):
    ws = _ws(_host(query, *dims), device)
    return ws, (_ptr(ws), ws.numel() * 8)


FPS_RESIDENT_MAX_N, FPS_RESIDENT_MAX_NPOINT = 16384, 15360


def furthest_point_sampling(xyz, npoint):
    _chk(xyz, "xyz", torch.float32, 3)
    B, N, _ = xyz.shape
    out = torch.empty((B, int(npoint)), dtype=torch.int32, device=xyz.device)
    if N <= FPS_RESIDENT_MAX_N and int(npoint) <= FPS_RESIDENT_MAX_NPOINT:
        _launch("ptt_fps_f32", xyz.device, _ptr(xyz), B, N, int(npoint), _ptr(out), timed='ptt_fps_f32')
    else:
        ws = torch.empty((B * N,), dtype=torch.float32, device=xyz.device)
        _launch("ptt_fps_ws_f32", xyz.device, _ptr(xyz), B, N, int(npoint), _ptr(out), _ptr(ws), ws.numel(), timed='ptt_fps_f32')
    return out


def gather_points(features, idx):
    _chk(features, "features", torch.float32, 3)
    _chk(idx, "idx", torch.int32, 2)
    B, C, N = features.shape
    M = idx.shape[1]
    out = torch.empty((B, C, M), dtype=torch.float32, device=features.device)
    _launch("ptt_gather_f32", features.device, _ptr(features), _ptr(idx), B, C, N, M, _ptr(out))
    return out


def scatter_add_det(src, idx, N):
    B, C, E = src.shape
    out = torch.empty((B, C, int(N)), dtype=torch.float32, device=src.device)
    nbytes = _host("ptt_scatter_add_det_workspace", B, int(N), E)
    ws = torch.empty((max(1, (nbytes + 3) // 4),), dtype=torch.int32, device=src.device)
    _launch("ptt_scatter_add_det_f32", src.device, _ptr(src), _ptr(idx), B, C, int(N), E, _ptr(out), _ptr(ws), ws.numel() * 4)
    return out


_ATOMIC_GRADS = os.environ.get("PTT_ATOMIC_GRADS", "0")


def set_atomic_grads(on):
    global _ATOMIC_GRADS
    prev = _ATOMIC_GRADS == "1"
    _ATOMIC_GRADS = "1" if on else "0"
    return prev


def _det_grads(entries, N):
    if int(N) * 16384 > 0xffffffff:
        return False
    return entries <= 16384 and _ATOMIC_GRADS != "1"


def gather_points_grad(grad_out, idx, N):
    _chk(grad_out, "grad_out", torch.float32, 3)
    _chk(idx, "idx", torch.int32, 2)
    B, C, M = grad_out.shape
    if M > 0 and _det_grads(M, N):
        return scatter_add_det(grad_out, idx, N)
    out = torch.empty((B, C, int(N)), dtype=torch.float32, device=grad_out.device)
    _launch("ptt_gather_grad_f32", grad_out.device, _ptr(grad_out), _ptr(idx), B, C, int(N), M, _ptr(out))
    return out


def select_centres(xyz, idx, npoint, want_idx64=True):
    _chk(xyz, "xyz", torch.float32, 3)
    B, N, _ = xyz.shape
    if idx is not None:
        _chk(idx, "idx", torch.int32, 2)
    new_xyz = torch.empty((B, int(npoint), 3), dtype=torch.float32, device=xyz.device)
    idx64 = torch.empty((B, int(npoint)), dtype=torch.int64, device=xyz.device) if (want_idx64 and idx is not None) else None
    _launch("ptt_select_centres_f32", xyz.device, _ptr(xyz), _ptr(idx), B, N, int(npoint), _ptr(new_xyz), _ptr(idx64))
    return new_xyz, idx64


GRID_BALL_QUERY_MIN_POINTS = 4096


def ball_query(new_xyz, xyz, radius, nsample):
    _chk(new_xyz, "new_xyz", torch.float32, 3)
    _chk(xyz, "xyz", torch.float32, 3)
    B, M, _ = new_xyz.shape
    N = xyz.shape[1]
    out = torch.empty((B, M, int(nsample)), dtype=torch.int32, device=xyz.device)
    if GRID_BALL_QUERY_MIN_POINTS <= N <= 131072:
        ws, ws_arg = _workspace("ptt_ball_query_grid_workspace", xyz.device, B, N)
        _launch("ptt_ball_query_grid_f32", xyz.device, _ptr(new_xyz), _ptr(xyz), B, M, N, float(radius), int(nsample), _ptr(out), *ws_arg,
# ... 761 lines not shown
            _ptr(bp), _ptr(out), cout, _ptr(part), part.numel(), timed='ptt_rows_gemm_f32')
    return out, part, dz


def bn_bwd_sums_from_partials(part):
    chunks, _, C = part.shape
    sums = torch.empty((2, C), dtype=torch.float64, device=part.device)
    _launch("ptt_bn_bwd_sums_partials_f64", part.device, _ptr(part), chunks, C, _ptr(sums))
    return sums


def bn_finish_partials(partials, rows, eps, bn=None):
    chunks, _, C = partials.shape
    mean, var, invstd = (torch.empty((C,), dtype=torch.float32, device=partials.device) for _ in range(3))
    if bn is not None:
        tail, a, b = _bn_tail(bn, C, partials.device)
        _launch("ptt_bn_finish_partials_train_f32", partials.device, _ptr(partials), chunks, C, int(rows), float(eps), _ptr(mean), _ptr(var),
                _ptr(invstd), ctypes.byref(tail))
        _bn_tail_done(bn)
        return mean, var, invstd, a, b
    _launch("ptt_bn_finish_partials_f32", partials.device, _ptr(partials), chunks, C, int(rows), float(eps), _ptr(mean), _ptr(var), _ptr(invstd))
    return mean, var, invstd


def bn_sums_partials(partials, rows):
    chunks, _, C = partials.shape
    sums = torch.empty((2 * C + 1,), dtype=torch.float64, device=partials.device)
    _launch("ptt_bn_sums_partials_f64", partials.device, _ptr(partials), chunks, C, int(rows), _ptr(sums))
    return sums


def colsum(x, out=None):
    _rows(x, "x")
    R, C = x.shape
    if R == 0:
        return x.sum(0) if out is None else out.zero_()
    if out is None:
        out = torch.empty((C,), dtype=torch.float32, device=x.device)
    ws, ws_arg = _workspace("ptt_colsum_workspace", x.device, R, C)
    _launch("ptt_colsum_f32", x.device, _ptr(x), R, C, x.stride(0), _ptr(out), *ws_arg)
    return out


def linear_wgrad(dz, x, out=None, accumulate=False, x_scale=None, x_shift=None):
    _rows(dz, "dz"); _rows(x, "x")
    R, Cout = dz.shape
    Cin = x.shape[1]
    if out is None:
        out = torch.empty((Cout, Cin), dtype=torch.float32, device=dz.device)
    ok2 = (dz.stride(0) % 4 == 0 and x.stride(0) % 4 == 0 and dz.data_ptr() % 16 == 0 and x.data_ptr() % 16 == 0
           and R * max(dz.stride(0), x.stride(0)) < (1 << 29))
    nb2 = _host("ptt_linear_wgrad2_workspace", R, Cout, Cin) if ok2 else 0
    two = bool(nb2 and WGRAD2)
    ws = _ws(nb2 if two else _host("ptt_linear_wgrad_workspace", R, Cout, Cin), dz.device)
    _launch("ptt_linear_wgrad2_f32" if two else "ptt_linear_wgrad_f32", dz.device, _ptr(dz), dz.stride(0), _ptr(x), x.stride(0), R, Cout, Cin,
            _ptr(out), int(bool(accumulate)), _ptr(ws), ws.numel() * 8, _ptr(x_scale), _ptr(x_shift), timed='ptt_linear_wgrad_f32')
    return out


def linear_wgrad_partials(dz, x, x_scale=None, x_shift=None):
    _rows(dz, "dz"); _rows(x, "x")
    R, Cout = dz.shape
    Cin = x.shape[1]
    ok2 = (dz.stride(0) % 4 == 0 and x.stride(0) % 4 == 0 and dz.data_ptr() % 16 == 0 and x.data_ptr() % 16 == 0
           and R * max(dz.stride(0), x.stride(0)) < (1 << 29))
    nb2 = _host("ptt_linear_wgrad2_workspace", R, Cout, Cin) if ok2 else 0
    nch = ctypes.c_int(0)
    two = bool(nb2 and WGRAD2)
    ws = _ws(nb2 if two else _host("ptt_linear_wgrad_workspace", R, Cout, Cin), dz.device)
    _launch("ptt_linear_wgrad2_partials_f32" if two else "ptt_linear_wgrad_partials_f32", dz.device, _ptr(dz), dz.stride(0), _ptr(x), x.stride(0),
            R, Cout, Cin, _ptr(ws), ws.numel() * 8, _ptr(x_scale), _ptr(x_shift), ctypes.byref(nch), timed='ptt_linear_wgrad_f32')
    return ws, nch.value


def colsum_partials(x):
    _rows(x, "x")
    R, C = x.shape
    ws, ws_arg = _workspace("ptt_colsum_workspace", x.device, R, C)
    nch = ctypes.c_int(0)
    _launch("ptt_colsum_partials_f32", x.device, _ptr(x), R, C, x.stride(0), *ws_arg, ctypes.byref(nch))
    return ws, nch.value


_capture_uploads = []


def finish_capture_uploads():
    done = []
    while _capture_uploads:
        table, host, keep = _capture_uploads.pop(0)
        table.copy_(host)
        done.append((table, keep))
    return done


class GradFinishPlan(object):

    def __init__(self, device):
        self.device = torch.device(device)
        self.signature = None
        self.capture_table = None
        self.uploaded = torch.cuda.Event()

    def prepare_capture(self):
        if self.signature is None:
            raise RuntimeError("GradFinishPlan: a step must have run eagerly before it is captured")
        self.capture_table = (torch.empty_like(self.table), torch.zeros(tuple(self.host.shape), dtype=torch.uint8))

    @staticmethod
    def _outputs_per_group(total_chunks):
        return 4 if total_chunks > 1024 else 8 if total_chunks > 256 else 16 if total_chunks > 64 else 32 if total_chunks > 8 else 64 if total_chunks > 2 else 256

    def _build(self, sig):
        by_dst, order = {}, []
        for k, (dst, cols, ld, n, nch) in enumerate(sig):
            key = (dst, cols, ld, n)
            if key not in by_dst:
                by_dst[key] = []
                order.append(key)
            by_dst[key].append(k)
        nseg = len(order)
        segs = (_lib.GradSegment * nseg)()
        blocks, self.job_order = [], []
        for si, key in enumerate(order):
            dst, cols, ld, n = key
            ks = by_dst[key]
            total = sum(sig[k][4] for k in ks)
            vec = int(n % 4 == 0 and cols % 4 == 0 and ld % 4 == 0 and dst % 4 == 0)
            out = self._outputs_per_group(total)
            segs[si] = _lib.GradSegment(dst=dst, n=n, cols=cols, ld=ld, job0=len(self.job_order), njobs=len(ks), out=out, vec=vec, reserved=0)
            self.job_order += ks
            units = n // 4 if vec else n
            for u in range(0, units, out):
                blocks += [si, u]
        spans = sorted((dst, dst + (n // cols - 1) * ld + cols, cols, ld) for dst, cols, ld, n in order)
        for (a0, a1, ac, al), (b0, b1, bc, bl) in zip(spans, spans[1:]):
            if b0 < a1 and not (al == bl and (b0 - a0) % al >= ac and (b0 - a0) % al + bc <= al):
                raise ValueError("GradFinishPlan: two gradient destinations overlap inside the flat buffer "
                                 "(elements %d..%d and %d..%d): the same parameter was handed over both whole and as a slice" % (a0, a1, b0, b1))
        self.vec_jobs = [bool(segs[si].vec) for si, key in enumerate(order) for _ in by_dst[key]]
        self.n_blocks = len(blocks) // 2
        self.segs = torch.frombuffer(bytearray(bytes(segs)), dtype=torch.uint8).to(self.device)
        self.blocks = torch.tensor(blocks, dtype=torch.int32, device=self.device)
        nj = len(self.job_order)
        self.host = torch.zeros((nj, ctypes.sizeof(_lib.GradJob)), dtype=torch.uint8).pin_memory()
        self.rows = (_lib.GradJob * nj).from_address(self.host.data_ptr())
        self.table = torch.empty_like(self.host, device=self.device)
        self.signature = sig

    def run(self, jobs, flat):
        if not jobs:
            return
        if flat.dtype != torch.float32 or not flat.is_contiguous() or flat.device != self.device or flat.data_ptr() % 16:
            raise ValueError("GradFinishPlan: a contiguous, 16-byte aligned float32 gradient buffer on %s expected" % self.device)
        total = flat.numel()
        sig = tuple((int(d), int(c), int(l), int(n), int(nch)) for d, c, l, n, _, nch in jobs)
        if sig != self.signature:
            for d, c, l, n, nch in sig:
                if n <= 0 or c <= 0 or n % c or l < c or nch <= 0 or d < 0 or d + (n // c - 1) * l + c > total:
                    raise ValueError("GradFinishPlan: job (dst %d, cols %d, ld %d, n %d, chunks %d) outside the %d-element buffer" % (d, c, l, n, nch, total))
            self._build(sig)
        capturing = torch.cuda.is_current_stream_capturing()
        if capturing:
            if sig != self.signature:
                raise RuntimeError("GradFinishPlan: a step must have run eagerly before it is captured (the segment tables are built then)")
            if self.capture_table is None:
                raise RuntimeError("GradFinishPlan: prepare_capture() must be called before the stream starts capturing")
            table, host = self.capture_table
            self.capture_table = None
            rows = (_lib.GradJob * len(self.job_order)).from_address(host.data_ptr())
            _capture_uploads.append((table, host, (self.segs, self.blocks)))
        else:
            self.uploaded.synchronize()
            rows, table = self.rows, self.table
        for r, k, vec in zip(rows, self.job_order, self.vec_jobs):
            ptr = int(jobs[k][4])
            if vec and ptr % 16:
                raise ValueError("GradFinishPlan: partial sums of a float4 segment must be 16-byte aligned")
            r.partial, r.nchunks = ptr, sig[k][4]
        if not capturing:
            self.table.copy_(self.host, non_blocking=True)
            self.uploaded.record()
        _launch("ptt_grad_finish_f32", self.device, _ptr(self.segs), _ptr(table), _ptr(self.blocks), self.n_blocks, _ptr(flat))


def pack_weight_strided(src, cout, k, stride_out, stride_k, batch, stride_batch):
    if not src.is_cuda or src.dtype != torch.float32:
        raise RuntimeError("src must be a float32 device tensor")
    n = _host("ptt_packed_weight_elems", int(cout), int(k))
    out = torch.empty((int(batch), n), dtype=torch.float32, device=src.device)
    _launch("ptt_pack_weight_strided_f32", src.device, _ptr(src), int(cout), int(k), int(stride_out), int(stride_k), int(batch), int(stride_batch),
            _ptr(out))
    return out


def pack_jobs_table(jobs, device):
    arr = (_lib.PackJob * len(jobs))()
    for n, (ptr, off, so, sk, cout, k) in enumerate(jobs):
        arr[n] = _lib.PackJob(W=ptr, out_offset=off, stride_out=so, stride_k=sk, Cout=cout, K=k)
    host = torch.frombuffer(bytearray(bytes(arr)), dtype=torch.uint8)
    return host.to(device)


def pack_weights(table, n_jobs, arena):
    if not arena.is_cuda or arena.dtype != torch.float32 or not arena.is_contiguous():
        raise RuntimeError("arena must be a contiguous float32 device tensor")
    _launch("ptt_pack_weights_f32", arena.device, _ptr(table), int(n_jobs), _ptr(arena))
    return arena


def linear_batched(x, wpacked, cout, residual=None):
    if not x.is_cuda or x.dtype != torch.float32 or x.dim() != 3 or x.stride(2) != 1:
        raise RuntimeError("x must be a (batch, rows, K) float32 device tensor with contiguous channels")
    Bt, rows, K = x.shape
    out = torch.empty((Bt, rows, int(cout)), dtype=torch.float32, device=x.device)
    r = residual
    if r is not None and (r.dim() != 3 or r.stride(2) != 1):
        raise RuntimeError("residual must be (batch, rows, cout) with contiguous channels")
    _launch("ptt_linear_batched_f32", x.device, _ptr(x), rows, K, x.stride(1), x.stride(0), _ptr(wpacked), wpacked.stride(0), int(cout), None, None,
            0, _ptr(r), r.stride(1) if r is not None else int(cout), r.stride(0) if r is not None else 0, _ptr(out), int(cout), rows * int(cout), Bt,
            timed='ptt_linear_f32')
    return out


def softmax_rows_(x, scale):
    _chk(x, "x", torch.float32)
    n = x.shape[-1]
    _launch("ptt_softmax_rows_f32", x.device, _ptr(x), x.numel() // n, n, n, float(scale))
    return x


def gather_rows(src, idx):
    _chk(src, "src", torch.float32, 3)
    _chk(idx, "idx", torch.int32, 2)
    B, N, C = src.shape
    E = idx.shape[1]
    out = torch.empty((B, E, C), dtype=torch.float32, device=src.device)
    _launch("ptt_gather_rows_f32", src.device, _ptr(src), _ptr(idx), B, N, E, C, _ptr(out))
    return out


def sa_z0_rows(xyz, new_xyz, idx, term, wx, radius, normalize_xyz, want_stats=False):
    _chk(xyz, "xyz", torch.float32, 3)
    _chk(new_xyz, "new_xyz", torch.float32, 3)
    _chk(idx, "idx", torch.int32, 3)
    if not (wx.is_cuda and wx.dtype == torch.float32 and wx.dim() == 2 and wx.stride(1) == 1):
        raise RuntimeError("wx must be a float32 (C,3) device tensor with unit column stride (a column slice of the weight is fine)")
    B, N, _ = xyz.shape
    _, M, ns = idx.shape
    C = wx.shape[0]
    if term is not None:
        _chk(term, "term", torch.float32, 3)
        if tuple(term.shape) != (B, N, C):
            raise RuntimeError("term must be (B,N,C) = %s, got %s" % ((B, N, C), tuple(term.shape)))
    if wx.shape[1] != 3 or new_xyz.shape[1] != M:
        raise RuntimeError("wx must be (C,3) and new_xyz (B,M,3)")
    z0 = torch.empty((B * M * ns, C), dtype=torch.float32, device=xyz.device)
    rel = torch.empty((B * M * ns, 3), dtype=torch.float32, device=xyz.device)
    chunks = _host("ptt_sa_z0_rows_stat_chunks", B, M, ns, C) if want_stats else 0
    if chunks:
        part = torch.empty((chunks, 2, C), dtype=torch.float64, device=xyz.device)
        _launch("ptt_sa_z0_rows_stats_f32", xyz.device, _ptr(xyz), _ptr(new_xyz), _ptr(idx), _ptr(term), _ptr(wx), wx.stride(0), B, N, M, ns, C,
                float(radius), int(bool(normalize_xyz)), _ptr(z0), _ptr(rel), _ptr(part), part.numel())
        return z0, rel, part
    _launch("ptt_sa_z0_rows_f32", xyz.device, _ptr(xyz), _ptr(new_xyz), _ptr(idx), _ptr(term), _ptr(wx), wx.stride(0), B, N, M, ns, C, float(radius),
            int(bool(normalize_xyz)), _ptr(z0), _ptr(rel))
# ... 446 lines not shown
```

### ptt_amd/train_ops.py

```python
import os
import weakref

import torch
import torch.distributed as dist
import torch.nn as nn

from . import ops


def _raw_pointer_ready(conv, bn, device):
    ts = [conv.weight] + ([conv.bias] if conv.bias is not None else [])
    if bn is not None:
        ts += [bn.weight, bn.bias, bn.running_mean, bn.running_var]
        nbt = bn.num_batches_tracked
        if nbt is not None and (nbt.dtype != torch.int64 or nbt.device != device):
            return False
    return all(t is not None and t.dtype == torch.float32 and t.device == device and t.is_contiguous() for t in ts)


def usable(mlp, x):
    if not (mlp.training and x.is_cuda and x.dtype == torch.float32 and len(mlp) > 0):
        return False
    for unit in mlp:
        conv = getattr(unit, 'conv', None)
# ... 131 lines not shown
                elems = self.plan.entries[k][1]
                self.cache[k] = self.arena[off:off + elems]
                off += elems
            hit = self.cache.get(ekey)
            if hit is not None:
                return hit
        w = W.detach()
        cout, k = (w.shape[1], w.shape[0]) if transpose else w.shape
        so, sk = (w.stride(1), w.stride(0)) if transpose else (w.stride(0), w.stride(1))
        hit = self.cache[ekey] = ops.pack_weight_strided(w, cout, k, so, sk, 1, 0)[0]
        return hit


def packed(W, transpose=False):
    if _pack_capture is not None:
        return _pack_capture.get(W, transpose)
    base = W._base if W._base is not None else W
    slot = _pack_slot(base)
    off = (W.data_ptr() - base.data_ptr())
    key = (off, tuple(W.shape), tuple(W.stride()), (W._version, base.data_ptr()), bool(transpose))
    hit = slot.get(key)
    if hit is not None:
        return hit
    ekey = (id(base), off, key[1], key[2], key[4])
    plan = _pack_plans.setdefault(W.device, _PackPlan()) if PACK_PLAN and W.dim() == 2 else None
    if plan is not None and ekey in plan.entries and plan.repack(W.device):
        hit = slot.get(key)
        if hit is not None:
            return hit
    for k in [k for k in slot if k[3] != key[3]]:
        del slot[k]
    w = W.detach()
    cout, k = (w.shape[1], w.shape[0]) if transpose else w.shape
    so, sk = (w.stride(1), w.stride(0)) if transpose else (w.stride(0), w.stride(1))
    hit = slot[key] = ops.pack_weight_strided(w, cout, k, so, sk, 1, 0)[0]
    if plan is not None:
        plan.register(ekey, base, hit.numel())
    return hit


def invalidate_packed():
    _pack_cache.clear()
    _pack_plans.clear()


def conv_rows(x, W2d, in_a=None, in_b=None, want_stats=False, transpose=False):
    cout, K = (W2d.shape[1], W2d.shape[0]) if transpose else W2d.shape
    wp = packed(W2d, transpose)
    if ops.rows_gemm_supported(x.shape[0], K, cout, x.stride(0), cout, x=x):
        if want_stats:
            return ops.rows_gemm(x, wp, cout, in_scale=in_a, in_shift=in_b, want_stats=True)
        return ops.rows_gemm(x, wp, cout, in_scale=in_a, in_shift=in_b), None
    z = ops.linear_act_in(x, in_a, in_b, wp, cout) if in_a is not None else ops.linear(x, wp, cout)
    return z, None


_row_counts = {}


def _row_count(rows, device):
    key = (int(rows), str(device))
    if key not in _row_counts:
        _row_counts[key] = torch.full((1,), float(rows), dtype=torch.float64, device=device)
    return _row_counts[key]


class GradSink(object):
    active = None

    def __init__(self, params, device):
        self.device = torch.device(device)
        self.params = [p for p in params if p.requires_grad]
        self.index, off = {}, 0
        for p in self.params:
            if not (p.is_cuda and p.device == self.device and p.dtype == torch.float32 and p.is_contiguous()):
                raise ValueError("GradSink: contiguous float32 parameters on %s expected" % self.device)
            if p.data_ptr() in self.index:
                raise ValueError("GradSink: two parameters share storage (tied weights): their gradients cannot be told apart by address")
            self.index[p.data_ptr()] = (off, p.numel())
            off += (p.numel() + 3) // 4 * 4
        self.flat = torch.zeros((max(off, 4),), dtype=torch.float32, device=self.device)
        self.views = [self.flat[self.index[p.data_ptr()][0]:self.index[p.data_ptr()][0] + p.numel()].view_as(p) for p in self.params]
        self.plan = ops.GradFinishPlan(self.device)
        self.jobs, self.keep = [], []
        self.attach()

    def attach(self):
        for p, v in zip(self.params, self.views):
            p.grad = v

    def collecting(self):
        sink = self

        class _Scope(object):
            def __enter__(self):
                if GradSink.active is not None:
                    raise RuntimeError("GradSink: another backward pass is being collected")
                if any(p.grad is not v for p, v in zip(sink.params, sink.views)):
                    sink.attach()
                sink.flat.zero_()
                sink.jobs, sink.keep = [], []
                GradSink.active = sink

            def __exit__(self, *exc):
                GradSink.active = None
                if exc[0] is not None:
                    sink.jobs, sink.keep = [], []
        return _Scope()

    def locate(self, w):
        if w is None:
            return None
        base = w._base if w._base is not None else w
        hit = self.index.get(base.data_ptr())
        if hit is None or hit[1] != base.numel():
            return None
        rel = (w.data_ptr() - base.data_ptr()) // 4
        n = w.numel()
        if n == 0 or rel < 0 or w.dtype != torch.float32:
            return None
        if w.is_contiguous():
            return (hit[0] + rel, n, n, n) if rel + n <= hit[1] else None
        if w.dim() == 2 and w.stride(1) == 1 and w.stride(0) >= w.shape[1] and rel + (w.shape[0] - 1) * w.stride(0) + w.shape[1] <= hit[1]:
            return (hit[0] + rel, w.shape[1], w.stride(0), n)
        return None

    def push(self, loc, partials, nchunks):
        self.jobs.append((loc[0], loc[1], loc[2], loc[3], partials.data_ptr(), int(nchunks)))
        self.keep.append(partials)

    def flush(self):
        self.plan.run(self.jobs, self.flat)
        self.jobs, self.keep = [], []


def _sunk(w):
    sink = GradSink.active
    loc = sink.locate(w) if sink is not None else None
    return (sink, loc) if loc is not None else (None, None)


def weight_grad(w, dz, x, x_scale=None, x_shift=None):
    sink, loc = _sunk(w)
    if sink is None:
        return ops.linear_wgrad(dz, x, x_scale=x_scale, x_shift=x_shift)
    ws, nch = ops.linear_wgrad_partials(dz, x, x_scale, x_shift)
    sink.push(loc, ws, nch)
    return None


def bias_grad(b, g2):
    sink, loc = _sunk(b)
    if sink is None:
        return ops.colsum(g2)
    ws, nch = ops.colsum_partials(g2)
    sink.push(loc, ws, nch)
    return None


def small_grad(p, g):
    if g is None:
        return None
    sink, loc = _sunk(p)
    if sink is None or g.numel() != loc[3] or g.dtype != torch.float32:
        return g
    g = g.contiguous()
    if g.data_ptr() % 16:
        g = g.clone()
    sink.push(loc, g, 1)
    return None


class _GatherRows(torch.autograd.Function):

    @staticmethod
    def forward(ctx, rows, idx):
        ctx.save_for_backward(idx)
        ctx.N = rows.shape[1]
        return ops.gather_rows(rows.contiguous(), idx)

    @staticmethod
    def backward(ctx, g):
        (idx,) = ctx.saved_tensors
        return ops.scatter_rows_det(g.contiguous(), idx, ctx.N), None


def gather_rows(rows, idx):
    return _GatherRows.apply(rows, idx)


class _AddRelTerm(torch.autograd.Function):

    @staticmethod
    def forward(ctx, gathered, rel, wx):
        ctx.save_for_backward(rel, wx)
        ctx.wx = wx
        return ops.linear(rel.contiguous(), packed(wx), wx.shape[0], residual=gathered.contiguous())

    @staticmethod
    def backward(ctx, g):
        rel, wx = ctx.saved_tensors
        g = g.contiguous()
        d_rel = ops.linear(g, packed(ctx.wx, True), 3) if ctx.needs_input_grad[1] else None
        d_wx = weight_grad(ctx.wx, g, rel.contiguous()) if ctx.needs_input_grad[2] else None
        return g, d_rel, d_wx


class _SplitCols(torch.autograd.Function):

    @staticmethod
    def forward(ctx, w, k):
        ctx.set_materialize_grads(False)
        ctx.w, ctx.k = w, int(k)
        return w[:, :k], w[:, k:]

    @staticmethod
    def backward(ctx, ga, gb):
        w, k = ctx.w, ctx.k
        ga, gb = small_grad(w[:, :k], ga), small_grad(w[:, k:], gb)
        if ga is None and gb is None:
            return None, None
        if ga is None:
            ga = gb.new_zeros((w.shape[0], k))
        if gb is None:
            gb = ga.new_zeros((w.shape[0], w.shape[1] - k))
        return torch.cat((ga, gb), dim=1), None


class _SharedMlpPool(torch.autograd.Function):

    @staticmethod
    def forward(ctx, x, ns, eps, preact, sync, bns, z0_part, front, f0, f1, f2, f3, f4, *params):
        ctx.set_materialize_grads(False)
        L = len(params) // 3
        saved, stats, counts = [], [], []
        ctx.front = front
        front_saved = ()
# ... 615 lines not shown
```

### ptt_amd/train_step.py

```python
import os
import warnings

import numpy as np
import torch
import torch.distributed as dist

from . import synth
from .optim import ClipAdam, _bump_versions

GRAD_ELEMS = 4903113


def synthetic_train_batch(seed, B, device, NS=1024, NT=512, K_s=200, K_t=100):
    s, t = synth.frames(seed, B, NS, NT, K_s=K_s, K_t=K_t)
    rs = np.random.RandomState(seed + 7919)
    cls = (rs.random_sample((B, NS)) > 0.7).astype(np.float32)
    reg = (rs.standard_normal((B, 4)) * 0.3).astype(np.float32)
    to = lambda a: torch.from_numpy(a).to(device)
    return {'search_points': to(s), 'template_points': to(t), 'batch_size': B, 'cls_label': to(cls), 'reg_label': to(reg)}


def broadcast_module_state(module, buffers_only=False, src=0):
    if not (dist.is_available() and dist.is_initialized()) or dist.get_world_size() == 1:
        return
# ... 53 lines not shown
        self.collective = collective
        self._collective_cfg = collective
        self.ddp = collective and reducer == "ddp"
        if sync_bn and self.world > 1:
            model = torch.nn.SyncBatchNorm.convert_sync_batchnorm(model)
        self.tracker = model
        if self.ddp:
            ids = [self.device.index] if self.device.type == 'cuda' else None
            self.model = torch.nn.parallel.DistributedDataParallel(model, device_ids=ids, bucket_cap_mb=bucket_cap_mb)
        else:
            self.model = model
        self.optimizer = ClipAdam(self.model.parameters(), lr=lr, betas=betas, eps=eps)
        self.clip = clip
        self.sink = None
        if reducer == "flat":
            from .train_ops import GradSink
            self.sink = GradSink(list(self.model.parameters()), self.device)
            if self.world > 1:
                self.sync_replicas()
        can_graph = reducer == "flat" and not (sync_bn and self.world > 1)
        if graph and not can_graph:
            raise ValueError("graph=True needs the flat reducer on a HIP device and no SyncBatchNorm exchange inside the step")
        self.graph_mode = can_graph and graph is not False and os.environ.get("PTT_TRAIN_GRAPH", "1") != "0"
        self.graph_warmup = max(1, int(graph_warmup))
        self.eager_steps = 0
        self.captured = None
        self.graph_steps = 0
        self._capture_misses = 0

    def sync_replicas(self, buffers_only=False):
        broadcast_module_state(self.tracker, buffers_only)

    def _local_forward_backward(self, batch):
        ret, _, _ = self.model(dict(batch))
        loss = ret['loss'] if ret['loss'].dim() == 0 else ret['loss'].mean()
        with self.sink.collecting():
            loss.backward()
        self.sink.flush()
        return loss

    def _reduce(self):
        dist.all_reduce(self.sink.flat)

    def forward_backward(self, batch):
        if self.sink is None:
            ret, _, _ = self.model(dict(batch))
            loss = ret['loss'] if ret['loss'].dim() == 0 else ret['loss'].mean()
            self.optimizer.zero_grad(set_to_none=True)
            loss.backward()
            return loss
        loss = self._local_forward_backward(batch)
        if self.collective:
            self._reduce()
            if self.world > 1:
                self.sink.flat.mul_(1.0 / self.world)
        return loss

    def step(self, batch):
        if self.graph_mode:
            if self.captured is not None and not self.captured.valid(self):
                self.captured = None
            if self.captured is None and self.eager_steps >= self.graph_warmup:
                self._capture(batch)
            if self.captured is not None and self.captured.accepts(batch):
                return self._replay(batch)
        loss = self.forward_backward(batch)
        self.optimizer.step(max_norm=self.clip if self.clip else None)
        self.tracker.update_global_step()
        self.eager_steps += 1
        return loss

    def _capture(self, batch):
        from . import ops, train_ops
        if not self.optimizer.prepare_graph_step():
            self._capture_misses += 1
            if self._capture_misses > 3:
                self.graph_mode = False
                warnings.warn("DataParallelTrainer: the optimizer is not in the one-table state a captured step needs; stepping eagerly")
            return
        self._capture_misses = 0
        clip = self.clip if self.clip else None
        cap = _CapturedStep(batch)
        try:
            self.sink.plan.prepare_capture()
            cap.packs = train_ops.PackCapture(list(self.model.parameters()), self.device)
            torch.cuda.synchronize(self.device)
            with cap.packs, torch.cuda.graph(cap.first, capture_error_mode="thread_local"):
                cap.loss = self._local_forward_backward(cap.static)
                if not self._collective_cfg:
                    self.optimizer.record_graph_step(clip)
            if self._collective_cfg:
                cap.second = torch.cuda.CUDAGraph()
                with cap.packs, torch.cuda.graph(cap.second, pool=cap.first.pool(), capture_error_mode="thread_local"):
                    if self.world > 1:
                        self.sink.flat.mul_(1.0 / self.world)
                    self.optimizer.record_graph_step(clip)
            cap.tables = ops.finish_capture_uploads()
        except Exception as e:
            ops.finish_capture_uploads()
            self.graph_mode = False
            warnings.warn("DataParallelTrainer: capturing the training step failed (%s: %s); stepping eagerly" % (type(e).__name__, e))
            return
        cap.optimizer_state = self.optimizer._graph
        cap.bn_buffers = [t for m in self.tracker.modules()
                          if isinstance(m, torch.nn.modules.batchnorm._BatchNorm) and m.training and m.track_running_stats
                          for t in (m.running_mean, m.running_var, m.num_batches_tracked) if t is not None]
        self.captured = cap

    def _replay(self, batch):
        cap = self.captured
        cap.load(batch)
        self.optimizer.begin_graph_step(self.clip if self.clip else None)
        cap.first.replay()
        if cap.second is not None:
            if self.collective:
                self._reduce()
            cap.second.replay()
        self.optimizer.end_graph_step()
        _bump_versions(cap.bn_buffers)
        self.tracker.update_global_step()
        self.graph_steps += 1
        return cap.loss

    def no_sync(self):
        if self.ddp:
            return self.model.no_sync()
        trainer = self

        class _Scope(object):
            def __enter__(self):
                self.was, trainer.collective = trainer.collective, False

            def __exit__(self, *exc):
                trainer.collective = self.was
        return _Scope()

    def grad_bytes_allreduced(self):
        if not self.collective:
            return 0
        return sum(p.numel() * p.element_size() for p in self.model.parameters() if p.requires_grad)

    def ranks_seen(self):
        if not self.collective:
            return 1
        one = torch.ones(1, device=self.device)
        dist.all_reduce(one)
        return int(one.item())
```

Before: 17480.

## Batch deferred weight-grad partials into one launch and pair search/template FPS

Weight-gradient and bias-column-sum partial computations are no longer launched one by one. They are queued as job descriptors and run at flush time by a single persistent-style kernel that dispatches each block to its job through a prefix table. Separately, a paired FPS kernel samples the search and template clouds in one launch, using 2B blocks. Both cut kernel-launch count and raise GPU occupancy for the many small training kernels. In exchange, the job kernel carries a 12-way template dispatch with register pressure set by the largest body, a linear job lookup per block, and delayed gradient computation that keeps operand tensors alive longer.

```diff
diff --git a/include/ptt_hip.h b/include/ptt_hip.h
--- a/include/ptt_hip.h
+++ b/include/ptt_hip.h
@@ -8,7 +8,7 @@
 extern "C" {
 #endif
 
-#define PTT_ABI_VERSION 26
+#define PTT_ABI_VERSION 27
 
 enum {
     PTT_OK = 0,
@@ -28,6 +28,9 @@
                 ptt_stream_t stream);
 int ptt_fps_ws_f32(const float* xyz, int B, int N, int npoint, int32_t* idx_out, float* workspace,
                    size_t workspace_elems, ptt_stream_t stream);
+int ptt_fps_pair_supported(int Na, int npoint_a, int Nb, int npoint_b);
+int ptt_fps_pair_f32(const float* xyz_a, int Na, int npoint_a, int32_t* idx_a, const float* xyz_b, int Nb, int npoint_b,
+                     int32_t* idx_b, int B, ptt_stream_t stream);
 
 int ptt_gather_f32(const float* feat, const int32_t* idx, int B, int C, int N, int M,
                    float* out, ptt_stream_t stream);
@@ -458,6 +461,27 @@
 int ptt_grad_finish_f32(const ptt_grad_segment* segments_device, const ptt_grad_job* jobs_device, const int32_t* blocks_device,
                         int n_blocks, float* flat, ptt_stream_t stream);
 
+#define PTT_GRAD_PART_WGRAD 0
+#define PTT_GRAD_PART_COLSUM 1
+typedef struct ptt_grad_part_job {
+    const float* dZ;
+    const float* X;
+    float* partial;
+    const float* x_scale;
+    const float* x_shift;
+    int32_t kind;
+    int32_t ldz, ldx, R, Cout, Cin;
+    int32_t nbi, chunk_rows, nchunks;
+    int32_t vz, vx, ns;
+    int32_t narrow_o, narrow_i;
+    int32_t grid_x, grid_y;
+} ptt_grad_part_job;
+int ptt_grad_part_wgrad_job(const float* dZ, int ldz, const float* X, int ldx, int R, int Cout, int Cin, void* workspace,
+                            size_t workspace_bytes, const float* x_scale, const float* x_shift, ptt_grad_part_job* job);
+int ptt_grad_part_colsum_job(const float* X, int R, int C, int ldx, void* workspace, size_t workspace_bytes, ptt_grad_part_job* job);
+int ptt_grad_jobs_f32(const ptt_grad_part_job* jobs_device, const int32_t* first_block_device, int njobs, int total_blocks,
+                      ptt_stream_t stream);
+
 int ptt_rows_gemm_rsum16_supported(int rows, int K, int N, int ldx);
 int ptt_rows_gemm_rsum16_f32(const float* X, int rows, int K, int ldx, const float* Wpacked, int N, const float* residual, int ldr,
                              float* out, int ldo, float* plain, int ldp, float* gsum, int ldg, ptt_stream_t stream);
diff --git a/ptt_amd/_lib.py b/ptt_amd/_lib.py
--- a/ptt_amd/_lib.py
+++ b/ptt_amd/_lib.py
@@ -140,6 +140,13 @@
 class GradSegment(Structure):
     _fields_ = [("dst", c_int64), ("n", c_int32), ("cols", c_int32), ("ld", c_int32), ("job0", c_int32), ("njobs", c_int32), ("out", c_int32),
                 ("vec", c_int32), ("reserved", c_int32)]
+
+
+class GradPartJob(Structure):
+    _fields_ = [("dZ", c_void_p), ("X", c_void_p), ("partial", c_void_p), ("x_scale", c_void_p), ("x_shift", c_void_p),
+                ("kind", c_int32), ("ldz", c_int32), ("ldx", c_int32), ("R", c_int32), ("Cout", c_int32), ("Cin", c_int32),
+                ("nbi", c_int32), ("chunk_rows", c_int32), ("nchunks", c_int32), ("vz", c_int32), ("vx", c_int32), ("ns", c_int32),
+                ("narrow_o", c_int32), ("narrow_i", c_int32), ("grid_x", c_int32), ("grid_y", c_int32)]
 
 
 class AdamHyper(Structure):
diff --git a/ptt_amd/csrc/point_ops.hip b/ptt_amd/csrc/point_ops.hip
--- a/ptt_amd/csrc/point_ops.hip
+++ b/ptt_amd/csrc/point_ops.hip
@@ -24,10 +24,8 @@
 
 
 template <int T, int P, bool LX, int ABL = 0>
-__global__ __launch_bounds__(T) void fps_kernel(const float* __restrict__ xyz, int N, int npoint,
-                                               int32_t* __restrict__ idx_out) {
+__device__ __forceinline__ void fps_body(const int b, const float* xyz, int N, int npoint, int32_t* idx_out) {
     constexpr int W = T / 64;
-    const int b = blockIdx.x;
     const float* __restrict__ pts = xyz + (size_t)b * N * 3;
     int32_t* __restrict__ out = idx_out + (size_t)b * npoint;
     const int t = threadIdx.x;
@@ -196,6 +194,20 @@
     for (int j = t; j < npoint; j += T) out[j] = sel_lds[j];
 }
 
+template <int T, int P, bool LX, int ABL = 0>
+__global__ __launch_bounds__(T) void fps_kernel(const float* __restrict__ xyz, int N, int npoint,
+                                               int32_t* __restrict__ idx_out) {
+    fps_body<T, P, LX, ABL>(blockIdx.x, xyz, N, npoint, idx_out);
+}
+
+template <int PA, int PB>
+__global__ __launch_bounds__(256) void fps_pair_kernel(const float* __restrict__ xyz_a, int Na, int npoint_a, int32_t* __restrict__ idx_a,
+                                                       const float* __restrict__ xyz_b, int Nb, int npoint_b, int32_t* __restrict__ idx_b,
+                                                       int B) {
+    if ((int)blockIdx.x < B) fps_body<256, PA, true>(blockIdx.x, xyz_a, Na, npoint_a, idx_a);
+    else fps_body<256, PB, true>(blockIdx.x - B, xyz_b, Nb, npoint_b, idx_b);
+}
+
 template <int T, int P>
 static int launch_fps(const float* xyz, int B, int N, int npoint, int32_t* idx, hipStream_t s) {
     const size_t sel_bytes = (size_t)((npoint + 3) & ~3) * sizeof(int);
@@ -1053,6 +1065,24 @@
     return fail(PTT_EUNSUPPORTED, "ptt_fps_f32: N=%d exceeds the register-resident limit 16384 (use ptt_fps_ws_f32)", N);
 }
 
+extern "C" int ptt_fps_pair_supported(int Na, int npoint_a, int Nb, int npoint_b) {
+    const size_t la = (size_t)((npoint_a + 3) & ~3) * 4 + (size_t)Na * 12, lb = (size_t)((npoint_b + 3) & ~3) * 4 + (size_t)Nb * 12;
+    return Na > 0 && Na <= 1024 && Nb > 0 && Nb <= 512 && npoint_a > 0 && npoint_b > 0 && la + 1024 <= 65536 && lb + 1024 <= 65536;
+}
+extern "C" int ptt_fps_pair_f32(const float* xyz_a, int Na, int npoint_a, int32_t* idx_a, const float* xyz_b, int Nb, int npoint_b,
+                                int32_t* idx_b, int B, ptt_stream_t stream) {
+    if (B < 0) return fail(PTT_EINVAL, "ptt_fps_pair_f32: B=%d", B);
+    if (!ptt_fps_pair_supported(Na, npoint_a, Nb, npoint_b))
+        return fail(PTT_EUNSUPPORTED, "ptt_fps_pair_f32: Na=%d npoint_a=%d Nb=%d npoint_b=%d (clouds of at most 1024 and 512 points)", Na,
+                    npoint_a, Nb, npoint_b);
+    if (B == 0) return PTT_OK;
+    if (!xyz_a || !idx_a || !xyz_b || !idx_b) return fail(PTT_EINVAL, "ptt_fps_pair_f32: null pointer");
+    const size_t la = (size_t)((npoint_a + 3) & ~3) * 4 + (size_t)Na * 12, lb = (size_t)((npoint_b + 3) & ~3) * 4 + (size_t)Nb * 12;
+    hipLaunchKernelGGL((fps_pair_kernel<4, 2>), dim3(2 * B), dim3(256), la > lb ? la : lb, as_stream(stream), xyz_a, Na, npoint_a, idx_a, xyz_b,
+                       Nb, npoint_b, idx_b, B);
+    return check_launch("fps_pair_kernel");
+}
+
 extern "C" int ptt_spatial_order_f32(const float* xyz, int B, int N, int32_t* order, ptt_stream_t stream) {
     if (B < 0 || N <= 0) return fail(PTT_EINVAL, "ptt_spatial_order_f32: B=%d N=%d", B, N);
     if (B == 0) return PTT_OK;
diff --git a/ptt_amd/csrc/train_ops.hip b/ptt_amd/csrc/train_ops.hip
--- a/ptt_amd/csrc/train_ops.hip
+++ b/ptt_amd/csrc/train_ops.hip
@@ -681,19 +681,19 @@
     }
 }
 
-template <bool VZ, bool VX, int NS = 1>
-__global__ __launch_bounds__(256, 2) void linear_wgrad_kernel(const float* __restrict__ dZ, int ldz, const float* __restrict__ X,
-                                                              int ldx, int R, int Cout, int Cin, int nbi, int chunk_rows,
-                                                              float* __restrict__ partial, const float* __restrict__ xa,
-                                                              const float* __restrict__ xb, int narrow_o = 0, int narrow_i = 0) {
+template <bool VZ, bool VX, int NS>
+__device__ __forceinline__ void linear_wgrad_body(const unsigned bx, const unsigned by, const float* __restrict__ dZ, int ldz,
+                                                  const float* __restrict__ X, int ldx, int R, int Cout, int Cin, int nbi, int chunk_rows,
+                                                  float* __restrict__ partial, const float* __restrict__ xa,
+                                                  const float* __restrict__ xb, int narrow_o, int narrow_i) {
     extern __shared__ __attribute__((aligned(16))) float wg_smem[];
     constexpr int WG_BUF = WG_KC * WG_LD;
 #define As(b) (wg_smem + (b) * WG_BUF)
 #define Bs(b) (wg_smem + (2 + (b)) * WG_BUF)
     const int t = threadIdx.x, lane = t & 63, w = t >> 6, half = lane >> 5, col = lane & 31;
-    const int bo = blockIdx.x / nbi, bi = blockIdx.x - bo * nbi;
+    const int bo = bx / nbi, bi = bx - bo * nbi;
     const int o0 = bo * 128, i0 = bi * 128;
-    const int r_begin = blockIdx.y * chunk_rows, r_end = min(R, r_begin + chunk_rows);
+    const int r_begin = by * chunk_rows, r_end = min(R, r_begin + chunk_rows);
     int wo = (w >> 1) * 64, wi = (w & 1) * 64;
     int sidx = 0;
     if constexpr (NS > 1) {
@@ -761,7 +761,7 @@
         __syncthreads();
         if (sidx != 0) return;
         const int step = (NS == 4) ? 1 : (narrow_i ? 1 : 2);
-        float* P = partial + (size_t)blockIdx.y * Cout * Cin;
+        float* P = partial + (size_t)by * Cout * Cin;
         for (int a = 0; a < 2; ++a)
             for (int b = 0; b < 2; ++b) {
                 const int ci = i0 + wi + b * 32 + col;
@@ -776,7 +776,7 @@
             }
         return;
     }
-    float* P = partial + (size_t)blockIdx.y * Cout * Cin;
+    float* P = partial + (size_t)by * Cout * Cin;
 #pragma unroll
     for (int a = 0; a < 2; ++a)
 #pragma unroll
@@ -790,17 +790,30 @@
         }
 }
 
-__global__ __launch_bounds__(256) void colsum_partial_scalar_kernel(const float* __restrict__ X, int ldx, int R, int C, int rows_per_chunk,
-                                                                    float* __restrict__ partial) {
-    __shared__ float red[4][64];
-    const int c = blockIdx.y * 64 + (threadIdx.x & 63), rg = threadIdx.x >> 6;
-    const int r0 = blockIdx.x * rows_per_chunk, r1 = min(R, r0 + rows_per_chunk);
+template <bool VZ, bool VX, int NS = 1>
+__global__ __launch_bounds__(256, 2) void linear_wgrad_kernel(const float* __restrict__ dZ, int ldz, const float* __restrict__ X,
+                                                              int ldx, int R, int Cout, int Cin, int nbi, int chunk_rows,
+                                                              float* __restrict__ partial, const float* __restrict__ xa,
+                                                              const float* __restrict__ xb, int narrow_o = 0, int narrow_i = 0) {
+    linear_wgrad_body<VZ, VX, NS>(blockIdx.x, blockIdx.y, dZ, ldz, X, ldx, R, Cout, Cin, nbi, chunk_rows, partial, xa, xb, narrow_o,
+                                  narrow_i);
+}
+
+__device__ __forceinline__ void colsum_partial_scalar_body(float (*red)[64], unsigned bx, unsigned by, const float* X, int ldx, int R,
+                                                           int C, int rows_per_chunk, float* partial) {
+    const int c = by * 64 + (threadIdx.x & 63), rg = threadIdx.x >> 6;
+    const int r0 = bx * rows_per_chunk, r1 = min(R, r0 + rows_per_chunk);
     float acc = 0.f;
     if (c < C)
         for (int r = r0 + rg; r < r1; r += 4) acc += X[(size_t)r * ldx + c];
     red[rg][threadIdx.x & 63] = acc;
     __syncthreads();
-    if (rg == 0 && c < C) partial[(size_t)blockIdx.x * C + c] = ((red[0][threadIdx.x] + red[1][threadIdx.x]) + red[2][threadIdx.x]) + red[3][threadIdx.x];
+    if (rg == 0 && c < C) partial[(size_t)bx * C + c] = ((red[0][threadIdx.x] + red[1][threadIdx.x]) + red[2][threadIdx.x]) + red[3][threadIdx.x];
+}
+__global__ __launch_bounds__(256) void colsum_partial_scalar_kernel(const float* __restrict__ X, int ldx, int R, int C, int rows_per_chunk,
+                                                                    float* __restrict__ partial) {
+    __shared__ float red[4][64];
+    colsum_partial_scalar_body(red, blockIdx.x, blockIdx.y, X, ldx, R, C, rows_per_chunk, partial);
 }
 
 constexpr int WK_ROWS = 256;
@@ -850,11 +863,10 @@
 }
 
 constexpr int CS_ROWS = 128;
-__global__ __launch_bounds__(256) void colsum_partial_kernel(const float* __restrict__ X, int ldx, int R, int C, int rows_per_chunk,
-                                                             float* __restrict__ partial) {
-    __shared__ f32x4t red[4][64];
-    const int q = blockIdx.y * 64 + (threadIdx.x & 63), rg = threadIdx.x >> 6;
-    const int r0 = blockIdx.x * rows_per_chunk, r1 = min(R, r0 + rows_per_chunk);
+__device__ __forceinline__ void colsum_partial_body(f32x4t (*red)[64], unsigned bx, unsigned by, const float* X, int ldx, int R, int C,
+                                                    int rows_per_chunk, float* partial) {
+    const int q = by * 64 + (threadIdx.x & 63), rg = threadIdx.x >> 6;
+    const int r0 = bx * rows_per_chunk, r1 = min(R, r0 + rows_per_chunk);
     f32x4t acc = {0.f, 0.f, 0.f, 0.f};
     if (4 * q < C) {
         int r = r0 + rg;
@@ -880,8 +892,38 @@
         for (int g = 1; g < 4; ++g)
 #pragma unroll
             for (int k = 0; k < 4; ++k) t[k] += red[g][threadIdx.x][k];
-        *reinterpret_cast<f32x4t*>(partial + (size_t)blockIdx.x * C + 4 * q) = t;
-    }
+        *reinterpret_cast<f32x4t*>(partial + (size_t)bx * C + 4 * q) = t;
+    }
+}
+__global__ __launch_bounds__(256) void colsum_partial_kernel(const float* __restrict__ X, int ldx, int R, int C, int rows_per_chunk,
+                                                             float* __restrict__ partial) {
+    __shared__ f32x4t red[4][64];
+    colsum_partial_body(red, blockIdx.x, blockIdx.y, X, ldx, R, C, rows_per_chunk, partial);
+}
+
+__global__ __launch_bounds__(256, 2) void grad_jobs_kernel(const ptt_grad_part_job* __restrict__ jobs, const int32_t* __restrict__ first_block,
+                                                           int njobs) {
+    extern __shared__ __attribute__((aligned(16))) float wg_smem[];
+    int j = 0;
+    while (j + 1 < njobs && (int)blockIdx.x >= first_block[j + 1]) ++j;
+    const ptt_grad_part_job jb = jobs[j];
+    const int local = (int)blockIdx.x - first_block[j];
+    const unsigned by = local / jb.grid_x, bx = local - by * jb.grid_x;
+    if (jb.kind == PTT_GRAD_PART_COLSUM) {
+        if (jb.vz) colsum_partial_body(reinterpret_cast<f32x4t(*)[64]>(wg_smem), bx, by, jb.dZ, jb.ldz, jb.R, jb.Cout, jb.chunk_rows, jb.partial);
+        else colsum_partial_scalar_body(reinterpret_cast<float(*)[64]>(wg_smem), bx, by, jb.dZ, jb.ldz, jb.R, jb.Cout, jb.chunk_rows, jb.partial);
+        return;
+    }
+#define PTT_JOB_CASE(VZ, VX, NS)                                                                                                       \
+    if (jb.vz == VZ && jb.vx == VX && jb.ns == NS) {                                                                                   \
+        linear_wgrad_body<VZ, VX, NS>(bx, by, jb.dZ, jb.ldz, jb.X, jb.ldx, jb.R, jb.Cout, jb.Cin, jb.nbi, jb.chunk_rows,      \
+                                      jb.partial, jb.x_scale, jb.x_shift, jb.narrow_o, jb.narrow_i);                                   \
+        return;                                                                                                                        \
+    }
+#define PTT_JOB_CASES(NS) PTT_JOB_CASE(1, 1, NS) PTT_JOB_CASE(1, 0, NS) PTT_JOB_CASE(0, 1, NS) PTT_JOB_CASE(0, 0, NS)
+    PTT_JOB_CASES(1) PTT_JOB_CASES(2) PTT_JOB_CASES(4)
+#undef PTT_JOB_CASES
+#undef PTT_JOB_CASE
 }
 
 template <int OUT>
@@ -1798,19 +1840,35 @@
     const int rows = colsum_rows_per_chunk(R, C);
     return (size_t)((R + rows - 1) / rows) * (size_t)C * sizeof(float);
 }
+static int colsum_job(const float* X, int R, int C, int ldx, float* out, void* ws, size_t ws_bytes, ptt_grad_part_job* jb) {
+    const int rows = colsum_rows_per_chunk(R, C), nch = (R + rows - 1) / rows;
+    if ((nch > 1 || !out) && (!ws || ws_bytes < ptt_colsum_workspace(R, C))) return fail(PTT_EWORKSPACE, "ptt_colsum_f32: workspace too small");
+    float* part = (nch == 1 && out) ? out : static_cast<float*>(ws);
+    const bool vec = !(C & 3) && !(ldx & 3) && !((reinterpret_cast<uintptr_t>(X) | reinterpret_cast<uintptr_t>(part)) & 15);
+    *jb = ptt_grad_part_job{};
+    jb->kind = PTT_GRAD_PART_COLSUM;
+    jb->dZ = X; jb->ldz = ldx; jb->R = R; jb->Cout = C; jb->partial = part;
+    jb->chunk_rows = rows; jb->nchunks = nch; jb->vz = vec;
+    jb->grid_x = nch; jb->grid_y = vec ? (C / 4 + 63) / 64 : (C + 63) / 64;
+    return PTT_OK;
+}
 static int colsum_run(const float* X, int R, int C, int ldx, float* out, void* ws, size_t ws_bytes, int* nchunks_out, ptt_stream_t stream) {
     if (R <= 0 || C <= 0 || ldx < C) return fail(PTT_EINVAL, "ptt_colsum_f32: R=%d C=%d ldx=%d", R, C, ldx);
     if (!X || (!out && !nchunks_out)) return fail(PTT_EINVAL, "ptt_colsum_f32: null pointer");
-    const int rows = colsum_rows_per_chunk(R, C), nch = (R + rows - 1) / rows;
+    ptt_grad_part_job jb;
+    if (int rc = colsum_job(X, R, C, ldx, out, ws, ws_bytes, &jb)) return rc;
     hipStream_t s2 = as_stream(stream);
-    if ((nch > 1 || !out) && (!ws || ws_bytes < ptt_colsum_workspace(R, C))) return fail(PTT_EWORKSPACE, "ptt_colsum_f32: workspace too small");
-    float* part = (nch == 1 && out) ? out : static_cast<float*>(ws);
-    const bool vec = !(C & 3) && !(ldx & 3) && !((reinterpret_cast<uintptr_t>(X) | reinterpret_cast<uintptr_t>(part)) & 15);
-    if (vec) hipLaunchKernelGGL(colsum_partial_kernel, dim3(nch, (C / 4 + 63) / 64), dim3(256), 0, s2, X, ldx, R, C, rows, part);
-    else hipLaunchKernelGGL(colsum_partial_scalar_kernel, dim3(nch, (C + 63) / 64), dim3(256), 0, s2, X, ldx, R, C, rows, part);
-    if (nch > 1 && out) launch_wgrad_finish(part, nch, (size_t)C, 0, out, s2);
+    const int nch = jb.nchunks;
+    if (jb.vz) hipLaunchKernelGGL(colsum_partial_kernel, dim3(jb.grid_x, jb.grid_y), dim3(256), 0, s2, X, ldx, R, C, jb.chunk_rows, jb.partial);
+    else hipLaunchKernelGGL(colsum_partial_scalar_kernel, dim3(jb.grid_x, jb.grid_y), dim3(256), 0, s2, X, ldx, R, C, jb.chunk_rows, jb.partial);
+    if (nch > 1 && out) launch_wgrad_finish(jb.partial, nch, (size_t)C, 0, out, s2);
     if (nchunks_out) *nchunks_out = nch;
     return check_launch("colsum_partial_kernel");
+}
+extern "C" int ptt_grad_part_colsum_job(const float* X, int R, int C, int ldx, void* ws, size_t ws_bytes, ptt_grad_part_job* job) {
+    if (!job) return fail(PTT_EINVAL, "ptt_grad_part_colsum_job: null pointer");
+    if (R <= 0 || C <= 0 || ldx < C || !X) return fail(PTT_EINVAL, "ptt_grad_part_colsum_job: R=%d C=%d ldx=%d or null pointer", R, C, ldx);
+    return colsum_job(X, R, C, ldx, nullptr, ws, ws_bytes, job);
 }
 extern "C" int ptt_colsum_f32(const float* X, int R, int C, int ldx, float* out, void* ws, size_t ws_bytes, ptt_stream_t stream) {
     if (!out) return fail(PTT_EINVAL, "ptt_colsum_f32: null pointer");
@@ -1828,17 +1886,45 @@
     return (size_t)((R + rows - 1) / rows) * (size_t)Cout * Cin * sizeof(float);
 }
 
-static int linear_wgrad_run(const float* dZ, int ldz, const float* X, int ldx, int R, int Cout, int Cin, float* dW,
-                            int accumulate, void* ws, size_t ws_bytes, const float* x_scale, const float* x_shift,
-                            int* nchunks_out, ptt_stream_t stream) {
+static int wgrad_check(const float* dZ, int ldz, const float* X, int ldx, int R, int Cout, int Cin, void* ws, size_t ws_bytes,
+                       const float* x_scale, const float* x_shift) {
     if (x_scale && (!x_shift || (Cin & 3) || ((reinterpret_cast<uintptr_t>(x_scale) | reinterpret_cast<uintptr_t>(x_shift)) & 15)))
         return fail(PTT_EINVAL, "ptt_linear_wgrad_f32: the input transform needs Cin %% 4 == 0 and 16-byte aligned scale / shift");
     if (R <= 0 || Cout <= 0 || Cin <= 0 || ldz < Cout || ldx < Cin)
         return fail(PTT_EINVAL, "ptt_linear_wgrad_f32: R=%d Cout=%d Cin=%d ldz=%d ldx=%d", R, Cout, Cin, ldz, ldx);
-    if (!dZ || !X || (!dW && !nchunks_out)) return fail(PTT_EINVAL, "ptt_linear_wgrad_f32: null pointer");
+    if (!dZ || !X) return fail(PTT_EINVAL, "ptt_linear_wgrad_f32: null pointer");
     if (!ws || ws_bytes < ptt_linear_wgrad_workspace(R, Cout, Cin))
         return fail(PTT_EWORKSPACE, "ptt_linear_wgrad_f32: workspace too small");
-    if (wgrad_smallk_ok(Cout, Cin) && !x_scale && (ldz & 3) == 0 && (reinterpret_cast<uintptr_t>(dZ) & 15) == 0) {
+    return PTT_OK;
+}
+static inline bool wgrad_takes_smallk(const float* dZ, int ldz, int Cout, int Cin, const float* x_scale) {
+    return wgrad_smallk_ok(Cout, Cin) && !x_scale && (ldz & 3) == 0 && (reinterpret_cast<uintptr_t>(dZ) & 15) == 0;
+}
+static void wgrad_job(const float* dZ, int ldz, const float* X, int ldx, int R, int Cout, int Cin, void* ws, const float* x_scale,
+                      const float* x_shift, ptt_grad_part_job* jb) {
+    const int rows = wgrad_chunk_rows(R, Cout, Cin);
+    const int nchunks = (R + rows - 1) / rows;
+    const int nbo = (Cout + 127) / 128, nbi = (Cin + 127) / 128;
+    const int narrow_o = (Cout <= 64), narrow_i = (Cin <= 64);
+    *jb = ptt_grad_part_job{};
+    jb->kind = PTT_GRAD_PART_WGRAD;
+    jb->dZ = dZ; jb->ldz = ldz; jb->X = X; jb->ldx = ldx; jb->R = R; jb->Cout = Cout; jb->Cin = Cin;
+    jb->partial = static_cast<float*>(ws); jb->x_scale = x_scale; jb->x_shift = x_shift;
+    jb->nbi = nbi; jb->chunk_rows = rows; jb->nchunks = nchunks;
+    jb->vz = (ldz & 3) == 0 && (reinterpret_cast<uintptr_t>(dZ) & 15) == 0;
+    jb->vx = (ldx & 3) == 0 && (reinterpret_cast<uintptr_t>(X) & 15) == 0;
+    jb->ns = (narrow_o ? 2 : 1) * (narrow_i ? 2 : 1);
+    jb->narrow_o = jb->ns > 1 ? narrow_o : 0; jb->narrow_i = jb->ns > 1 ? narrow_i : 0;
+    jb->grid_x = nbo * nbi; jb->grid_y = nchunks;
+}
+constexpr int WG_LDS_BYTES = 4 * WG_KC * WG_LD * (int)sizeof(float);
+
+static int linear_wgrad_run(const float* dZ, int ldz, const float* X, int ldx, int R, int Cout, int Cin, float* dW,
+                            int accumulate, void* ws, size_t ws_bytes, const float* x_scale, const float* x_shift,
+                            int* nchunks_out, ptt_stream_t stream) {
+    if (int rc = wgrad_check(dZ, ldz, X, ldx, R, Cout, Cin, ws, ws_bytes, x_scale, x_shift)) return rc;
+    if (!dW && !nchunks_out) return fail(PTT_EINVAL, "ptt_linear_wgrad_f32: null pointer");
+    if (wgrad_takes_smallk(dZ, ldz, Cout, Cin, x_scale)) {
         const int nch = (R + WK_ROWS - 1) / WK_ROWS;
         hipStream_t s2 = as_stream(stream);
         float* part = static_cast<float*>(ws);
@@ -1858,29 +1944,28 @@
         if (nchunks_out) *nchunks_out = nch;
         return check_launch("wgrad_stream_kernel");
     }
-    const int rows = wgrad_chunk_rows(R, Cout, Cin);
-    const int nchunks = (R + rows - 1) / rows;
-    const int nbo = (Cout + 127) / 128, nbi = (Cin + 127) / 128;
+    ptt_grad_part_job jb;
+    wgrad_job(dZ, ldz, X, ldx, R, Cout, Cin, ws, x_scale, x_shift, &jb);
+    const int nchunks = jb.nchunks, nbi = jb.nbi, rows = jb.chunk_rows;
     hipStream_t s = as_stream(stream);
-    const int lds = 4 * WG_KC * WG_LD * (int)sizeof(float);
-    const bool vz = (ldz & 3) == 0 && (reinterpret_cast<uintptr_t>(dZ) & 15) == 0;
-    const bool vx = (ldx & 3) == 0 && (reinterpret_cast<uintptr_t>(X) & 15) == 0;
-    const int narrow_o = (Cout <= 64), narrow_i = (Cin <= 64);
-    const int ns = (narrow_o ? 2 : 1) * (narrow_i ? 2 : 1);
+    const int lds = WG_LDS_BYTES;
+    const bool vz = jb.vz, vx = jb.vx;
+    const int ns = jb.ns;
+    const dim3 grid(jb.grid_x, jb.grid_y);
 #define PTT_WGRAD_CASE(VZ, VX)                                                                                        \
     if (vz == VZ && vx == VX) {                                                                                       \
         if (ns == 1) {                                                                                                \
             if (int rc = set_lds_limit(reinterpret_cast<const void*>(linear_wgrad_kernel<VZ, VX, 1>), lds)) return rc; \
-            hipLaunchKernelGGL((linear_wgrad_kernel<VZ, VX, 1>), dim3(nbo * nbi, nchunks), dim3(256), lds, s, dZ, ldz, X, ldx, R, Cout, \
+            hipLaunchKernelGGL((linear_wgrad_kernel<VZ, VX, 1>), grid, dim3(256), lds, s, dZ, ldz, X, ldx, R, Cout,   \
                                Cin, nbi, rows, static_cast<float*>(ws), x_scale, x_shift, 0, 0);                      \
         } else if (ns == 2) {                                                                                         \
             if (int rc = set_lds_limit(reinterpret_cast<const void*>(linear_wgrad_kernel<VZ, VX, 2>), lds)) return rc; \
-            hipLaunchKernelGGL((linear_wgrad_kernel<VZ, VX, 2>), dim3(nbo * nbi, nchunks), dim3(256), lds, s, dZ, ldz, X, ldx, R, Cout, \
-                               Cin, nbi, rows, static_cast<float*>(ws), x_scale, x_shift, narrow_o, narrow_i);        \
+            hipLaunchKernelGGL((linear_wgrad_kernel<VZ, VX, 2>), grid, dim3(256), lds, s, dZ, ldz, X, ldx, R, Cout,   \
+                               Cin, nbi, rows, static_cast<float*>(ws), x_scale, x_shift, jb.narrow_o, jb.narrow_i);  \
         } else {                                                                                                      \
             if (int rc = set_lds_limit(reinterpret_cast<const void*>(linear_wgrad_kernel<VZ, VX, 4>), lds)) return rc; \
-            hipLaunchKernelGGL((linear_wgrad_kernel<VZ, VX, 4>), dim3(nbo * nbi, nchunks), dim3(256), lds, s, dZ, ldz, X, ldx, R, Cout, \
-                               Cin, nbi, rows, static_cast<float*>(ws), x_scale, x_shift, narrow_o, narrow_i);        \
+            hipLaunchKernelGGL((linear_wgrad_kernel<VZ, VX, 4>), grid, dim3(256), lds, s, dZ, ldz, X, ldx, R, Cout,   \
+                               Cin, nbi, rows, static_cast<float*>(ws), x_scale, x_shift, jb.narrow_o, jb.narrow_i);  \
         }                                                                                                             \
     }
     PTT_WGRAD_CASE(true, true) PTT_WGRAD_CASE(true, false) PTT_WGRAD_CASE(false, true) PTT_WGRAD_CASE(false, false)
@@ -1888,6 +1973,24 @@
     if (dW) launch_wgrad_finish(static_cast<const float*>(ws), nchunks, (size_t)Cout * Cin, accumulate, dW, s);
     if (nchunks_out) *nchunks_out = nchunks;
     return check_launch("linear_wgrad_kernel");
+}
+extern "C" int ptt_grad_part_wgrad_job(const float* dZ, int ldz, const float* X, int ldx, int R, int Cout, int Cin, void* ws,
+                                       size_t ws_bytes, const float* x_scale, const float* x_shift, ptt_grad_part_job* job) {
+    if (!job) return fail(PTT_EINVAL, "ptt_grad_part_wgrad_job: null pointer");
+    if (int rc = wgrad_check(dZ, ldz, X, ldx, R, Cout, Cin, ws, ws_bytes, x_scale, x_shift)) return rc;
+    *job = ptt_grad_part_job{};
+    if (wgrad_takes_smallk(dZ, ldz, Cout, Cin, x_scale) || wgrad_stream_ok(R, Cout, Cin, ldz, ldx)) return PTT_OK;
+    wgrad_job(dZ, ldz, X, ldx, R, Cout, Cin, ws, x_scale, x_shift, job);
+    return PTT_OK;
+}
+extern "C" int ptt_grad_jobs_f32(const ptt_grad_part_job* jobs_device, const int32_t* first_block_device, int njobs, int total_blocks,
+                                 ptt_stream_t stream) {
+    if (njobs < 0 || total_blocks < 0) return fail(PTT_EINVAL, "ptt_grad_jobs_f32: njobs=%d total_blocks=%d", njobs, total_blocks);
+    if (njobs == 0 || total_blocks == 0) return PTT_OK;
+    if (!jobs_device || !first_block_device) return fail(PTT_EINVAL, "ptt_grad_jobs_f32: null table");
+    if (int rc = set_lds_limit(reinterpret_cast<const void*>(grad_jobs_kernel), WG_LDS_BYTES)) return rc;
+    hipLaunchKernelGGL(grad_jobs_kernel, dim3(total_blocks), dim3(256), WG_LDS_BYTES, as_stream(stream), jobs_device, first_block_device, njobs);
+    return check_launch("grad_jobs_kernel");
 }
 extern "C" int ptt_linear_wgrad_f32(const float* dZ, int ldz, const float* X, int ldx, int R, int Cout, int Cin, float* dW,
                                     int accumulate, void* ws, size_t ws_bytes, const float* x_scale, const float* x_shift,
diff --git a/ptt_amd/models/backbones_3d/pointnet2_backbone.py b/ptt_amd/models/backbones_3d/pointnet2_backbone.py
--- a/ptt_amd/models/backbones_3d/pointnet2_backbone.py
+++ b/ptt_amd/models/backbones_3d/pointnet2_backbone.py
@@ -5,6 +5,8 @@
 
 from ... import graph_policy, ops, train_ops
 from .pointnet2 import pointnet2_modules
+
+FPS_PAIR = True
 
 
 class PointNet2BackboneLight(nn.Module):
@@ -109,11 +111,20 @@
         return (pointnet2_utils.furthest_point_sample(search_points[..., 0:3].contiguous(), sa.NPOINTS_SEARCH[0]),
                 pointnet2_utils.furthest_point_sample(template_points[..., 0:3].contiguous(), sa.NPOINTS_TEMPLATE[0]))
 
+    def sample_pair(self, search_points, template_points):
+        sa = self.model_cfg.SA_CONFIG
+        s, t = search_points[..., 0:3].contiguous(), template_points[..., 0:3].contiguous()
+        if sa.SAMPLE_METHOD[0] != 'fps' or not ops.fps_pair_supported(s, sa.NPOINTS_SEARCH[0], t, sa.NPOINTS_TEMPLATE[0]):
+            return None
+        return ops.fps_pair(s, sa.NPOINTS_SEARCH[0], t, sa.NPOINTS_TEMPLATE[0])
+
     def forward_branches(self, search_points, template_points, inds=None):
         sa = self.model_cfg.SA_CONFIG
         i_s, i_t = inds if inds is not None else (None, None)
         last = (len(self.SA_modules) - 1,) if (search_points.is_cuda and not self.training) else ()
         if not (self.overlap_branches and search_points.is_cuda and not self.training):
+            if inds is None and FPS_PAIR and self.training and search_points.is_cuda and search_points.dtype == torch.float32:
+                i_s, i_t = self.sample_pair(search_points, template_points) or (None, None)
             r = self.branch_forward(search_points, sa.NPOINTS_SEARCH, i_s, want_knn=self.seed_knn, compact_levels=last)
             t_seeds, t_feats, t_inds = self.branch_forward(template_points, sa.NPOINTS_TEMPLATE, i_t)
         else:
diff --git a/ptt_amd/ops.py b/ptt_amd/ops.py
--- a/ptt_amd/ops.py
+++ b/ptt_amd/ops.py
@@ -146,6 +146,24 @@
 
 
 FPS_RESIDENT_MAX_N, FPS_RESIDENT_MAX_NPOINT = 16384, 15360
+
+
+def fps_pair_supported(xyz_a, npoint_a, xyz_b, npoint_b):
+    return bool(xyz_a.is_cuda and xyz_b.is_cuda and xyz_a.dim() == xyz_b.dim() == 3 and xyz_a.shape[0] == xyz_b.shape[0]
+                and _host("ptt_fps_pair_supported", xyz_a.shape[1], int(npoint_a), xyz_b.shape[1], int(npoint_b)))
+
+
+def fps_pair(xyz_a, npoint_a, xyz_b, npoint_b):
+    _chk(xyz_a, "xyz_a", torch.float32, 3)
+    _chk(xyz_b, "xyz_b", torch.float32, 3)
+    B = xyz_a.shape[0]
+    if xyz_b.shape[0] != B:
+        raise RuntimeError("fps_pair: both sets must hold the same number of clouds")
+    out_a = torch.empty((B, int(npoint_a)), dtype=torch.int32, device=xyz_a.device)
+    out_b = torch.empty((B, int(npoint_b)), dtype=torch.int32, device=xyz_a.device)
+    _launch("ptt_fps_pair_f32", xyz_a.device, _ptr(xyz_a), xyz_a.shape[1], int(npoint_a), _ptr(out_a), _ptr(xyz_b), xyz_b.shape[1], int(npoint_b),
+            _ptr(out_b), B, timed='ptt_fps_f32')
+    return out_a, out_b
 
 
 def furthest_point_sampling(xyz, npoint):
@@ -1073,6 +1091,30 @@
     return ws, nch.value
 
 
+def wgrad_part_job(dz, x, x_scale=None, x_shift=None):
+    _rows(dz, "dz"); _rows(x, "x")
+    R, Cout = dz.shape
+    Cin = x.shape[1]
+    ok2 = (dz.stride(0) % 4 == 0 and x.stride(0) % 4 == 0 and dz.data_ptr() % 16 == 0 and x.data_ptr() % 16 == 0
+           and R * max(dz.stride(0), x.stride(0)) < (1 << 29))
+    if ok2 and WGRAD2 and _host("ptt_linear_wgrad2_workspace", R, Cout, Cin):
+        return None
+    ws = _ws(_host("ptt_linear_wgrad_workspace", R, Cout, Cin), dz.device)
+    job = _lib.GradPartJob()
+    _host_checked("ptt_grad_part_wgrad_job", _ptr(dz), dz.stride(0), _ptr(x), x.stride(0), R, Cout, Cin, _ptr(ws), ws.numel() * 8, _ptr(x_scale),
+                  _ptr(x_shift), ctypes.byref(job))
+    return (job, ws) if job.grid_x else None
+
+
+def colsum_part_job(x):
+    _rows(x, "x")
+    R, C = x.shape
+    ws, ws_arg = _workspace("ptt_colsum_workspace", x.device, R, C)
+    job = _lib.GradPartJob()
+    _host_checked("ptt_grad_part_colsum_job", _ptr(x), R, C, x.stride(0), *ws_arg, ctypes.byref(job))
+    return job, ws
+
+
 _capture_uploads = []
 
 
@@ -1173,6 +1215,59 @@
             self.table.copy_(self.host, non_blocking=True)
             self.uploaded.record()
         _launch("ptt_grad_finish_f32", self.device, _ptr(self.segs), _ptr(table), _ptr(self.blocks), self.n_blocks, _ptr(flat))
+
+
+class GradJobsPlan(object):
+
+    def __init__(self, device):
+        self.device = torch.device(device)
+        self.njobs = 0
+        self.host = self.table = None
+        self.capture_table = None
+        self.uploaded = torch.cuda.Event()
+
+    @staticmethod
+    def _bytes(njobs):
+        return njobs * ctypes.sizeof(_lib.GradPartJob) + (njobs + 1) * 4
+
+    def prepare_capture(self):
+        if self.njobs:
+            nb = self._bytes(self.njobs)
+            self.capture_table = (torch.empty((nb,), dtype=torch.uint8, device=self.device), torch.zeros((nb,), dtype=torch.uint8))
+
+    def run(self, jobs):
+        if not jobs:
+            return
+        jobs = sorted(jobs, key=lambda j: (j.kind, -j.chunk_rows))
+        nj, nb = len(jobs), self._bytes(len(jobs))
+        capturing = torch.cuda.is_current_stream_capturing()
+        if capturing:
+            if self.capture_table is None or self.capture_table[0].numel() != nb:
+                raise RuntimeError("GradJobsPlan: prepare_capture() after an eager step of the same shapes must precede the capture")
+            table, host = self.capture_table
+            self.capture_table = None
+            _capture_uploads.append((table, host, ()))
+        else:
+            if self.host is None or self.host.numel() < nb:
+                self.uploaded.synchronize()
+                self.host = torch.zeros((2 * nb,), dtype=torch.uint8).pin_memory()
+                self.table = torch.empty_like(self.host, device=self.device)
+            self.uploaded.synchronize()
+            table, host = self.table, self.host
+        rows = (_lib.GradPartJob * nj).from_address(host.data_ptr())
+        first = (ctypes.c_int32 * (nj + 1)).from_address(host.data_ptr() + nj * ctypes.sizeof(_lib.GradPartJob))
+        total = 0
+        for k, j in enumerate(jobs):
+            rows[k] = j
+            first[k] = total
+            total += j.grid_x * j.grid_y
+        first[nj] = total
+        if not capturing:
+            table[:nb].copy_(host[:nb], non_blocking=True)
+            self.uploaded.record()
+        self.njobs = nj
+        _launch("ptt_grad_jobs_f32", self.device, _ptr(table), ctypes.c_void_p(table.data_ptr() + nj * ctypes.sizeof(_lib.GradPartJob)), nj, total,
+                timed='ptt_grad_jobs_f32')
 
 
 def pack_weight_strided(src, cout, k, stride_out, stride_k, batch, stride_batch):
diff --git a/ptt_amd/train_ops.py b/ptt_amd/train_ops.py
--- a/ptt_amd/train_ops.py
+++ b/ptt_amd/train_ops.py
@@ -237,7 +237,8 @@
         self.flat = torch.zeros((max(off, 4),), dtype=torch.float32, device=self.device)
         self.views = [self.flat[self.index[p.data_ptr()][0]:self.index[p.data_ptr()][0] + p.numel()].view_as(p) for p in self.params]
         self.plan = ops.GradFinishPlan(self.device)
-        self.jobs, self.keep = [], []
+        self.part_plan = ops.GradJobsPlan(self.device)
+        self.jobs, self.keep, self.queued = [], [], []
         self.attach()
 
     def attach(self):
@@ -254,13 +255,13 @@
                 if any(p.grad is not v for p, v in zip(sink.params, sink.views)):
                     sink.attach()
                 sink.flat.zero_()
-                sink.jobs, sink.keep = [], []
+                sink.jobs, sink.keep, sink.queued = [], [], []
                 GradSink.active = sink
 
             def __exit__(self, *exc):
                 GradSink.active = None
                 if exc[0] is not None:
-                    sink.jobs, sink.keep = [], []
+                    sink.jobs, sink.keep, sink.queued = [], [], []
         return _Scope()
 
     def locate(self, w):
@@ -284,9 +285,23 @@
         self.jobs.append((loc[0], loc[1], loc[2], loc[3], partials.data_ptr(), int(nchunks)))
         self.keep.append(partials)
 
+    def queue(self, loc, made, *operands):
+        job, ws = made
+        self.queued.append(job)
+        self.keep.extend(t for t in operands if t is not None)
+        self.push(loc, ws, job.nchunks)
+
+    def prepare_capture(self):
+        self.plan.prepare_capture()
+        self.part_plan.prepare_capture()
+
     def flush(self):
+        self.part_plan.run(self.queued)
         self.plan.run(self.jobs, self.flat)
-        self.jobs, self.keep = [], []
+        self.jobs, self.keep, self.queued = [], [], []
+
+
+DEFER_PARTIALS = True
 
 
 def _sunk(w):
@@ -299,6 +314,10 @@
     sink, loc = _sunk(w)
     if sink is None:
         return ops.linear_wgrad(dz, x, x_scale=x_scale, x_shift=x_shift)
+    made = ops.wgrad_part_job(dz, x, x_scale, x_shift) if DEFER_PARTIALS else None
+    if made is not None:
+        sink.queue(loc, made, dz, x, x_scale, x_shift)
+        return None
     ws, nch = ops.linear_wgrad_partials(dz, x, x_scale, x_shift)
     sink.push(loc, ws, nch)
     return None
@@ -308,6 +327,9 @@
     sink, loc = _sunk(b)
     if sink is None:
         return ops.colsum(g2)
+    if DEFER_PARTIALS:
+        sink.queue(loc, ops.colsum_part_job(g2), g2)
+        return None
     ws, nch = ops.colsum_partials(g2)
     sink.push(loc, ws, nch)
     return None
diff --git a/ptt_amd/train_step.py b/ptt_amd/train_step.py
--- a/ptt_amd/train_step.py
+++ b/ptt_amd/train_step.py
@@ -159,7 +159,7 @@
         clip = self.clip if self.clip else None
         cap = _CapturedStep(batch)
         try:
-            self.sink.plan.prepare_capture()
+            self.sink.prepare_capture()
             cap.packs = train_ops.PackCapture(list(self.model.parameters()), self.device)
             torch.cuda.synchronize(self.device)
             with cap.packs, torch.cuda.graph(cap.first, capture_error_mode="thread_local"):
```

Result: no change. 17460 (-0.1%).
